# sergivalverde/sub-cortical_segmentation

Measured on NVIDIA B200. Metric: voxels_per_sec_full_volume_inference, higher is better.
Workload: dtype bf16

## Files before the change

sub-cortical_segmentation_b200/csrc/conv_sweep.cu:

```cuda
#include "tc_common.cuh"

namespace sc {

constexpr int SW_SLOT_HALF = 17408;
constexpr int SW_MAX_SLOTS = 14;
constexpr int SW_BAR_BYTES = 512;

struct SweepArgs {
  int Pw, R;
  int bn;
  int S;
  int nstrips, strip_w;
  int nseg, L;
  int n_items;
  int stages;
  int out_bufs;
  int npanels;
  int in_dx, in_dy;
  const float* scale; const float* shift; const float* alpha;
  unsigned long long* dbg;
  const uint8_t* item_on;
  double* stats;
  int st_H, st_pitch;
};

__device__ __forceinline__ void sweep_mma(uint32_t acc, uint32_t a_lo, uint32_t b_lo, uint32_t idesc, uint32_t accumulate, uint32_t elected) {
  asm volatile(
      "{\n\t"
      ".reg .pred p, q;\n\t"
      ".reg .b64 da, db;\n\t"
      "setp.ne.b32 p, %4, 0;\n\t"
      "setp.ne.b32 q, %5, 0;\n\t"
      "mov.b64 da, {%1, %6};\n\t"
      "mov.b64 db, {%2, %6};\n\t"
      "@q tcgen05.mma.cta_group::1.kind::f16 [%0], da, db, %3, p;\n\t"
      "}" ::"r"(acc), "r"(a_lo), "r"(b_lo), "r"(idesc), "r"(accumulate), "r"(elected), "r"(0x40004040u) : "memory");
}
__device__ __forceinline__ uint32_t desc_lo(uint32_t saddr) { return ((saddr & 0x3FFFFu) >> 4) | (1u << 16); }

__device__ __forceinline__ void tmem_ld16(uint32_t taddr, uint32_t (&r)[16]) {
  asm volatile(
      "tcgen05.ld.sync.aligned.32x32b.x16.b32 {%0, %1, %2, %3, %4, %5, %6, %7, %8, %9, %10, %11, %12, %13, %14, %15}, [%16];"
      : "=r"(r[0]), "=r"(r[1]), "=r"(r[2]), "=r"(r[3]), "=r"(r[4]), "=r"(r[5]), "=r"(r[6]), "=r"(r[7]), "=r"(r[8]),
        "=r"(r[9]), "=r"(r[10]), "=r"(r[11]), "=r"(r[12]), "=r"(r[13]), "=r"(r[14]), "=r"(r[15])
      : "r"(taddr));
}

__device__ __forceinline__ void tmem_ld8(uint32_t taddr, uint32_t (&r)[8]) {
  asm volatile("tcgen05.ld.sync.aligned.32x32b.x8.b32 {%0, %1, %2, %3, %4, %5, %6, %7}, [%8];"
               : "=r"(r[0]), "=r"(r[1]), "=r"(r[2]), "=r"(r[3]), "=r"(r[4]), "=r"(r[5]), "=r"(r[6]), "=r"(r[7])
               : "r"(taddr));
}
template <int CW>
__device__ __forceinline__ void sweep_stats_flush(float (&st_s)[CW], float (&st_q)[CW], float* s_red , int ew, int c0,
                                                  bool real, int lane, double* stats) {
#pragma unroll
  for (int k = 0; k < CW; ++k)
#pragma unroll
    for (int o = 16; o; o >>= 1) { st_s[k] += __shfl_xor_sync(0xffffffffu, st_s[k], o); st_q[k] += __shfl_xor_sync(0xffffffffu, st_q[k], o); }
  if (lane == 0) {
#pragma unroll
    for (int k = 0; k < CW; ++k) { s_red[ew * 2 * CW + k] = st_s[k]; s_red[ew * 2 * CW + CW + k] = st_q[k]; }
  }
  asm volatile("bar.sync 7, 512;" ::: "memory");
  if ((ew & 3) == 0 && real && lane < 2 * CW) {
    const int base = ew * 2 * CW + lane;
    const float tot = s_red[base] + s_red[base + 2 * CW] + s_red[base + 4 * CW] + s_red[base + 6 * CW];
    const int mom = lane / CW, ch = c0 + (lane - mom * CW);
    if (ch < 64) atomicAdd(&stats[ch * 2 + mom], (double)tot);
  }
}

template <int CW>
__device__ __forceinline__ void tmem_ld(uint32_t taddr, uint32_t (&r)[CW]) {
  if constexpr (CW == 16) tmem_ld16(taddr, r); else tmem_ld8(taddr, r);
}
template <int CW>
__device__ __forceinline__ void tmem_zero(uint32_t taddr) {
  if constexpr (CW == 16)
    asm volatile("tcgen05.st.sync.aligned.32x32b.x16.b32 [%0], {%1, %1, %1, %1, %1, %1, %1, %1, %1, %1, %1, %1, %1, %1, %1, %1};"
                 ::"r"(taddr), "r"(0u) : "memory");
  else
    asm volatile("tcgen05.st.sync.aligned.32x32b.x8.b32 [%0], {%1, %1, %1, %1, %1, %1, %1, %1};" ::"r"(taddr), "r"(0u) : "memory");
}
template <int CW>
__device__ __forceinline__ void sweep_acc_clear(uint32_t tcol, int S, int bn) {
  for (int j = 0; j < S + 2; ++j) tmem_zero<CW>(tcol + (uint32_t)(j * bn));
  asm volatile("tcgen05.wait::st.sync.aligned;" ::: "memory");
}
template <int CW, bool PAIR>
__device__ __forceinline__ void sweep_drain(uint64_t* afull, uint64_t* aempty, uint32_t& dj, uint32_t& dph, int S, int bn,
                                            uint32_t tcol, bool real, bool keep, int lane, float (&acc)[CW], bool timed,
                                            uint32_t& w_wait) {
  const long long c0 = timed ? clock64() : 0;
  mbar_wait(&afull[dj], (dph >> dj) & 1u);
  dph ^= 1u << dj;
  if (timed) w_wait += (uint32_t)(clock64() - c0);
  asm volatile("tcgen05.fence::after_thread_sync;" ::: "memory");
  if (real) {
    const uint32_t taddr = tcol + dj * (uint32_t)bn, tspill = taddr + (uint32_t)(S * bn);
    const bool split = dj < 2;
    if (keep) {
#pragma unroll
      for (int h = 0; h < CW; h += 8) {
        uint32_t r1[8], r2[8];
        tmem_ld8(taddr + h, r1);
        if (split) tmem_ld8(tspill + h, r2);
        asm volatile("tcgen05.wait::ld.sync.aligned;" ::: "memory");
#pragma unroll
        for (int k = 0; k < 8; ++k) acc[h + k] = split ? __uint_as_float(r1[k]) + __uint_as_float(r2[k]) : __uint_as_float(r1[k]);
      }
    }
    tmem_zero<CW>(taddr);
    if (split) tmem_zero<CW>(tspill);
    asm volatile("tcgen05.wait::st.sync.aligned;" ::: "memory");
  }
  asm volatile("tcgen05.fence::before_thread_sync;" ::: "memory");
  __syncwarp();
  if (lane == 0) {
    if (PAIR) mbar_arrive_cta(&aempty[dj], 0); else mbar_arrive(&aempty[dj]);
  }
  if (++dj == (uint32_t)S) dj = 0;
}
__device__ __forceinline__ void sweep_claim(uint64_t* aempty, uint32_t j, uint32_t& eph) {
  mbar_wait(&aempty[j], ((eph >> j) & 1u) ^ 1u);
  eph ^= 1u << j;
}
__device__ __forceinline__ uint32_t slot_back(uint32_t j, uint32_t k, int S) { return j >= k ? j - k : j + (uint32_t)S - k; }
__device__ __forceinline__ void tma_store_3d(const CUtensorMap* map, const void* src, int c0, int c1, int c2) {
  asm volatile("cp.async.bulk.tensor.3d.global.shared::cta.bulk_group [%0, {%2, %3, %4}], [%1];"
               ::"l"(reinterpret_cast<uint64_t>(map)), "r"(smem_u32(src)), "r"(c0), "r"(c1), "r"(c2) : "memory");
}
template <int KSTEPS, int DIL, int POOL, int CW, bool LO64, bool OUT32>
__global__ void __launch_bounds__(576, 1)
conv_sweep_kernel(const __grid_constant__ CUtensorMap mapA, const __grid_constant__ CUtensorMap mapW, const __grid_constant__ CUtensorMap mapO,
                  const SweepArgs a) {
  extern __shared__ uint8_t smem_raw[];
  uint8_t* smem = smem_raw + ((1024u - (smem_u32(smem_raw) & 1023u)) & 1023u);
  constexpr int BOXPX = 128 + 2 * DIL;
  constexpr int BOX_BYTES = BOXPX * 128;
  constexpr int NBOX = LO64 ? 1 : 2;
  constexpr int SLOT = NBOX * SW_SLOT_HALF;
  constexpr int LO_OFF = LO64 ? 64 : SW_SLOT_HALF;
  const int half_bytes = 3 * a.bn * 128;
  const int panel_bytes = 2 * half_bytes;
  const int w_bytes = a.npanels * panel_bytes;
  uint8_t* sW = smem;
  uint8_t* sRing = smem + w_bytes;
  constexpr int OB_BYTES = OUT32 ? 16384 : 32768;
  uint8_t* sOut = sRing + a.stages * SLOT;
  uint64_t* bars = reinterpret_cast<uint64_t*>(sOut + a.out_bufs * OB_BYTES);
  uint64_t* full = bars;
  uint64_t* empty = bars + a.stages;
  uint64_t* afull = bars + 2 * a.stages;
  uint64_t* aempty = afull + a.S;
  uint64_t* wfull = aempty + a.S;
  uint32_t* tmem_slot = reinterpret_cast<uint32_t*>(wfull + 1);
  float* s_const = reinterpret_cast<float*>(tmem_slot + 2);
  float* s_xch = s_const + 192;

  const int warp = threadIdx.x >> 5, lane = threadIdx.x & 31;

  if (threadIdx.x == 0) {
    for (int s = 0; s < a.stages; ++s) { mbar_init(&full[s], 1); mbar_init(&empty[s], 1); }
    for (int j = 0; j < a.S; ++j) { mbar_init(&afull[j], 1); mbar_init(&aempty[j], 16); }
    mbar_init(wfull, 1);
    asm volatile("fence.mbarrier_init.release.cluster;" ::: "memory");
  }
  if (warp == 1) {
    asm volatile("tcgen05.alloc.cta_group::1.sync.aligned.shared::cta.b32 [%0], %1;" ::"r"(smem_u32(tmem_slot)), "r"(512) : "memory");
    asm volatile("tcgen05.relinquish_alloc_permit.cta_group::1.sync.aligned;" ::: "memory");
  }
  for (int i = threadIdx.x; i < 64; i += blockDim.x) {
    const bool ok = i < a.bn;
    s_const[i] = ok ? __ldg(a.scale + i) : 0.f;
    s_const[64 + i] = ok ? __ldg(a.shift + i) : 0.f;
    s_const[128 + i] = ok ? __ldg(a.alpha + i) : 0.f;
  }
  for (int i = threadIdx.x; i < a.out_bufs * OB_BYTES / 16; i += blockDim.x)
    reinterpret_cast<uint4*>(sOut)[i] = make_uint4(0u, 0u, 0u, 0u);
  asm volatile("fence.proxy.async.shared::cta;" ::: "memory");
  asm volatile("tcgen05.fence::before_thread_sync;" ::: "memory");
  __syncthreads();
  asm volatile("tcgen05.fence::after_thread_sync;" ::: "memory");
  const uint32_t tmem_base = *tmem_slot;
  const int q4 = warp & 3, ew = warp - 2, grp = ew >> 2, c0 = grp * CW;
  const bool real = c0 < a.bn;
  const uint32_t tcol = tmem_base + ((uint32_t)(q4 * 32) << 16) + (uint32_t)c0;
  if (warp >= 2 && real) sweep_acc_clear<CW>(tcol, a.S, a.bn);
  asm volatile("tcgen05.fence::before_thread_sync;" ::: "memory");
  __syncthreads();
  asm volatile("tcgen05.fence::after_thread_sync;" ::: "memory");

  auto decode = [&](int item, int& w0, int& q, int& n0, int& Lc) {
    const int strip = item % a.nstrips;
    const int rest = item / a.nstrips;
    q = rest % DIL;
    const int seg = rest / DIL;
    w0 = strip * a.strip_w;
    const int Nq = (a.R - q + DIL - 1) / DIL;
    n0 = seg * a.L;
    Lc = Nq - n0 < a.L ? Nq - n0 : a.L;
  };

  if (warp == 0) {
    if (lane == 0) {
      asm volatile("prefetch.tensormap [%0];" ::"l"(reinterpret_cast<uint64_t>(&mapA)) : "memory");
      asm volatile("prefetch.tensormap [%0];" ::"l"(reinterpret_cast<uint64_t>(&mapW)) : "memory");
      asm volatile("prefetch.tensormap [%0];" ::"l"(reinterpret_cast<uint64_t>(&mapO)) : "memory");
      mbar_expect_tx(wfull, (uint32_t)w_bytes);
      for (int p = 0; p < 2 * a.npanels; ++p) tma_load_2d(&mapW, wfull, sW + p * half_bytes, 0, p * 3 * a.bn);
      uint32_t g = 0;
      long long w_empty = 0;
      const long long tstart = a.dbg ? clock64() : 0;
      for (int item = blockIdx.x; item < a.n_items; item += gridDim.x) {
        int w0, q, n0, Lc;
        decode(item, w0, q, n0, Lc);
        if (Lc <= 0 || (a.item_on && !a.item_on[item])) continue;
        const int nload = Lc + (POOL == 1 ? 1 : 0) + 2;
        for (int m = 0; m < nload; ++m, ++g) {
          const uint32_t s = g % a.stages, use = g / a.stages;
          if (use > 0) {
            const long long c0 = a.dbg ? clock64() : 0;
            mbar_wait(&empty[s], (use - 1) & 1);
            if (a.dbg) w_empty += clock64() - c0;
          }
          mbar_expect_tx(&full[s], (uint32_t)(NBOX * BOX_BYTES));
          uint8_t* sp = sRing + s * SLOT;
          const int r = q + DIL * (n0 + m);
          tma_load_3d(&mapA, &full[s], sp, 0, w0 + a.in_dx, r + a.in_dy);
          if (NBOX == 2) tma_load_3d(&mapA, &full[s], sp + SW_SLOT_HALF, 64, w0 + a.in_dx, r + a.in_dy);
        }
      }
      if (a.dbg) { a.dbg[blockIdx.x * 8 + 0] = (unsigned long long)w_empty; a.dbg[blockIdx.x * 8 + 1] = (unsigned long long)(clock64() - tstart); }
    }
    __syncwarp();
  } else if (warp == 1) {
    const uint32_t leader = elect_one();
    const uint32_t idesc = (1u << 4) | (1u << 7) | (1u << 10) | ((uint32_t)(3 * a.bn >> 3) << 17) | ((uint32_t)(128 >> 4) << 24);
    mbar_wait(wfull, 0);
    const uint32_t w_lo = desc_lo(smem_u32(sW));
    const uint32_t ring_lo = desc_lo(smem_u32(sRing));
    const uint32_t panel16 = (uint32_t)(panel_bytes >> 4), wl_off = (uint32_t)(half_bytes >> 4);
    uint32_t rs = 0, rph = 0;
    uint32_t j = 2, eph = 0;
    bool open = false;
    long long w_full = 0, w_tempty = 0;
    const long long tstart = a.dbg ? clock64() : 0;
    for (int item = blockIdx.x; item < a.n_items; item += gridDim.x) {
      int w0, q, n0, Lc;
      decode(item, w0, q, n0, Lc);
      if (Lc <= 0 || (a.item_on && !a.item_on[item])) continue;
      const int nin = Lc + (POOL == 1 ? 1 : 0) + 2;
      const uint32_t j0 = (uint32_t)(n0 + 2) % (uint32_t)a.S;
      const uint32_t d = open ? (j0 + (uint32_t)a.S - j) % (uint32_t)a.S : 2u;
      if (d) {
        if (open && leader) { umma_commit(&afull[slot_back(j, 2, a.S)]); if (d >= 2) umma_commit(&afull[slot_back(j, 1, a.S)]); }
        if (d >= 2) sweep_claim(aempty, slot_back(j0, 2, a.S), eph);
        sweep_claim(aempty, slot_back(j0, 1, a.S), eph);
      }
      j = j0; open = true;
      for (int m = 0; m < nin; ++m) {
        long long c0 = a.dbg ? clock64() : 0;
        sweep_claim(aempty, j, eph);
        if (a.dbg) { const long long c1 = clock64(); w_tempty += c1 - c0; c0 = c1; }
        mbar_wait(&full[rs], rph);
        if (a.dbg) w_full += clock64() - c0;
        asm volatile("tcgen05.fence::after_thread_sync;" ::: "memory");
        const uint32_t p = slot_back(j, 2, a.S);
        const uint32_t acc = tmem_base + p * (uint32_t)a.bn;
        const uint32_t sl = ring_lo + rs * (SLOT >> 4);
#pragma unroll
        for (int kx = 0; kx < 3; ++kx) {
#pragma unroll
          for (int ks = 0; ks < KSTEPS; ++ks) {
            const int gk = kx * KSTEPS + ks;
            const uint32_t a_hi = sl + (uint32_t)(kx * DIL * 8 + ks * 2);
            const uint32_t a_lo = a_hi + (uint32_t)(LO_OFF >> 4);
            const uint32_t wh = w_lo + (uint32_t)(gk >> 2) * panel16 + (uint32_t)((gk & 3) * 2);
            sweep_mma(acc, a_lo, wh, idesc, 1, leader);
            sweep_mma(acc, a_hi, wh + wl_off, idesc, 1, leader);
            sweep_mma(acc, a_hi, wh, idesc, 1, leader);
          }
        }
        if (leader) {
          umma_commit(&empty[rs]);
          umma_commit(&afull[p]);
        }
        __syncwarp();
        if (++rs == (uint32_t)a.stages) { rs = 0; rph ^= 1; }
        if (++j == (uint32_t)a.S) j = 0;
      }
    }
    if (open && leader) {
      umma_commit(&afull[slot_back(j, 2, a.S)]);
      umma_commit(&afull[slot_back(j, 1, a.S)]);
    }
    __syncwarp();
    if (a.dbg && leader) {
      a.dbg[blockIdx.x * 8 + 2] = (unsigned long long)w_full; a.dbg[blockIdx.x * 8 + 3] = (unsigned long long)w_tempty;
      a.dbg[blockIdx.x * 8 + 4] = (unsigned long long)(clock64() - tstart);
    }
  } else {
    const int px = q4 * 32 + lane;
    const bool issuer = threadIdx.x == 64;
    const int trow = POOL == 2 ? px >> 1 : px;
    const bool writer = POOL == 2 ? !(lane & 1) : true;
    const uint32_t row_off = (uint32_t)trow * 128u;
    const uint32_t sw = (uint32_t)(trow & 7);
    const uint32_t hi_chunk = (uint32_t)(c0 >> 3);
    const uint32_t lo_base = OUT32 ? 0u : 16384u, lo_chunk = OUT32 ? 4u + hi_chunk : hi_chunk;
    uint32_t t = 0, e = 0;
    uint32_t dj = 0, dph = 0;
    uint32_t w_tfull = 0;
    const bool timed = a.dbg != nullptr;
    const long long tstart = a.dbg ? clock64() : 0;
    constexpr bool STATS = POOL == 0 && DIL == 1;
    float st_s[STATS ? CW : 1], st_q[STATS ? CW : 1];
#pragma unroll
    for (int k = 0; k < (STATS ? CW : 1); ++k) st_s[k] = st_q[k] = 0.f;
    float v[CW];
    for (int item = blockIdx.x; item < a.n_items; item += gridDim.x) {
      int w0, q, n0, Lc;
      decode(item, w0, q, n0, Lc);
      if (Lc <= 0 || (a.item_on && !a.item_on[item])) continue;
      const int nrow = Lc + (POOL == 1 ? 1 : 0);
      const uint32_t j0 = (uint32_t)(n0 + 2) % (uint32_t)a.S;
      const uint32_t d = (j0 + 2u * (uint32_t)a.S - 2u - dj) % (uint32_t)a.S;
      if (t == 0 || d >= 3) {
        if (t > 0)
          for (int h = 0; h < 2; ++h) sweep_drain<CW, false>(afull, aempty, dj, dph, a.S, a.bn, tcol, real, false, lane, v, timed, w_tfull);
        dj = slot_back(j0, 2, a.S);
      } else {
        for (uint32_t h = 0; h < d; ++h) sweep_drain<CW, false>(afull, aempty, dj, dph, a.S, a.bn, tcol, real, false, lane, v, timed, w_tfull);
      }
      for (int h = 0; h < 2; ++h) sweep_drain<CW, false>(afull, aempty, dj, dph, a.S, a.bn, tcol, real, false, lane, v, timed, w_tfull);
      float hprev[CW];
#pragma unroll
      for (int k = 0; k < CW; ++k) hprev[k] = 0.f;
      for (int m = 0; m < nrow; ++m, ++t) {
        sweep_drain<CW, false>(afull, aempty, dj, dph, a.S, a.bn, tcol, real, true, lane, v, timed, w_tfull);
        if (real) {
#pragma unroll
          for (int k4 = 0; k4 < CW / 4; ++k4) {
            const float4 sc_ = *reinterpret_cast<const float4*>(s_const + c0 + 4 * k4);
            const float4 sh = *reinterpret_cast<const float4*>(s_const + 64 + c0 + 4 * k4);
            const float4 al = *reinterpret_cast<const float4*>(s_const + 128 + c0 + 4 * k4);
            v[4 * k4 + 0] = prelu(fmaf(v[4 * k4 + 0], sc_.x, sh.x), al.x);
            v[4 * k4 + 1] = prelu(fmaf(v[4 * k4 + 1], sc_.y, sh.y), al.y);
            v[4 * k4 + 2] = prelu(fmaf(v[4 * k4 + 2], sc_.z, sh.z), al.z);
            v[4 * k4 + 3] = prelu(fmaf(v[4 * k4 + 3], sc_.w, sh.w), al.w);
          }
        }

        int r_out = q + DIL * (n0 + m);
        if (POOL == 1) {
          if (real) {
            float* xw = s_xch + (((t & 1) * 4 + grp) * 4 + q4) * 32;
            if (lane < DIL) {
#pragma unroll
              for (int k4 = 0; k4 < CW / 4; ++k4)
                *reinterpret_cast<float4*>(xw + lane * 16 + 4 * k4) = make_float4(v[4 * k4], v[4 * k4 + 1], v[4 * k4 + 2], v[4 * k4 + 3]);
            }
            asm volatile("bar.sync %0, 128;" ::"r"(1 + grp) : "memory");
            const bool edge = lane >= 32 - DIL;
            const float* xr = s_xch + (((t & 1) * 4 + grp) * 4 + ((q4 + 1) & 3)) * 32 + (edge ? (lane - (32 - DIL)) * 16 : 0);
#pragma unroll
            for (int k4 = 0; k4 < CW / 4; ++k4) {
              const float4 x4 = *reinterpret_cast<const float4*>(xr + 4 * k4);
              const float xs[4] = {x4.x, x4.y, x4.z, x4.w};
#pragma unroll
              for (int k = 0; k < 4; ++k) {
                float nb = __shfl_down_sync(0xffffffffu, v[4 * k4 + k], DIL);
                if (edge) nb = xs[k];
                const float h = fmaxf(v[4 * k4 + k], nb);
                v[4 * k4 + k] = fmaxf(h, hprev[4 * k4 + k]);
                hprev[4 * k4 + k] = h;
              }
            }
          }
          if (m == 0) continue;
          r_out -= DIL;
        }
        if (POOL == 2) {
          if (real) {
#pragma unroll
            for (int k = 0; k < CW; ++k) {
              const float h = fmaxf(v[k], __shfl_down_sync(0xffffffffu, v[k], 1));
              v[k] = fmaxf(h, hprev[k]);
              hprev[k] = (m & 1) ? 0.f : h;
            }
          }
          if (!(m & 1)) continue;
          r_out >>= 1;
        }
        if constexpr (STATS) {
          if (a.stats && real) {
            const int wpx = w0 + px;
            if (wpx < a.Pw && (wpx & (a.st_pitch - 1)) < a.st_H && r_out < a.st_H) {
#pragma unroll
              for (int k = 0; k < CW; ++k) { st_s[k] += v[k]; st_q[k] = fmaf(v[k], v[k], st_q[k]); }
            }
          }
        }
        uint8_t* ob = sOut + (e % (uint32_t)a.out_bufs) * OB_BYTES;
        if (a.out_bufs == 1) {
          if (issuer) asm volatile("cp.async.bulk.wait_group.read 0;" ::: "memory");
          asm volatile("bar.sync 5, 512;" ::: "memory");
        }
        if (real) {
          uint32_t hi[CW / 2], lo[CW / 2];
#pragma unroll
          for (int k = 0; k < CW / 2; ++k) split2(v[2 * k], v[2 * k + 1], hi[k], lo[k]);
#pragma unroll
          for (int c = 0; c < CW / 8; ++c) {
            if (!writer) break;
            *reinterpret_cast<uint4*>(ob + row_off + (((hi_chunk + c) ^ sw) << 4)) = make_uint4(hi[4 * c], hi[4 * c + 1], hi[4 * c + 2], hi[4 * c + 3]);
            *reinterpret_cast<uint4*>(ob + lo_base + row_off + (((lo_chunk + c) ^ sw) << 4)) = make_uint4(lo[4 * c], lo[4 * c + 1], lo[4 * c + 2], lo[4 * c + 3]);
          }
          asm volatile("fence.proxy.async.shared::cta;" ::: "memory");
        }
        if (a.out_bufs == 2 && issuer) asm volatile("cp.async.bulk.wait_group.read 0;" ::: "memory");
        asm volatile("bar.sync 6, 512;" ::: "memory");
        if (issuer) {
          tma_store_3d(&mapO, ob, 0, POOL == 2 ? w0 >> 1 : w0, r_out);
          if (!OUT32) tma_store_3d(&mapO, ob + 16384, 64, POOL == 2 ? w0 >> 1 : w0, r_out);
          asm volatile("cp.async.bulk.commit_group;" ::: "memory");
        }
        ++e;
      }
    }
    if (t > 0)
      for (int h = 0; h < 2; ++h) sweep_drain<CW, false>(afull, aempty, dj, dph, a.S, a.bn, tcol, real, false, lane, v, timed, w_tfull);
    if (issuer) asm volatile("cp.async.bulk.wait_group 0;" ::: "memory");
    if constexpr (STATS) {
      if (a.stats) sweep_stats_flush<CW>(st_s, st_q, s_xch, ew, c0, real, lane, a.stats);
    }
    if (a.dbg && threadIdx.x == 64) {
      a.dbg[blockIdx.x * 8 + 5] = (unsigned long long)w_tfull; a.dbg[blockIdx.x * 8 + 6] = (unsigned long long)(clock64() - tstart);
      a.dbg[blockIdx.x * 8 + 7] = t;
    }
  }
  asm volatile("tcgen05.fence::before_thread_sync;" ::: "memory");
  __syncthreads();
  if (warp == 1) {
    asm volatile("tcgen05.fence::after_thread_sync;" ::: "memory");
    asm volatile("tcgen05.dealloc.cta_group::1.sync.aligned.b32 %0, %1;" ::"r"(tmem_base), "r"(512) : "memory");
  }
}

__device__ __forceinline__ void sweep_mma_2sm(uint32_t acc, uint32_t a_lo, uint32_t b_lo, uint32_t idesc, uint32_t accumulate, uint32_t elected) {
  asm volatile(
      "{\n\t"
      ".reg .pred p, q;\n\t"
      ".reg .b64 da, db;\n\t"
      "setp.ne.b32 p, %4, 0;\n\t"
      "setp.ne.b32 q, %5, 0;\n\t"
      "mov.b64 da, {%1, %6};\n\t"
      "mov.b64 db, {%2, %6};\n\t"
      "@q tcgen05.mma.cta_group::2.kind::f16 [%0], da, db, %3, p;\n\t"
      "}" ::"r"(acc), "r"(a_lo), "r"(b_lo), "r"(idesc), "r"(accumulate), "r"(elected), "r"(0x40004040u) : "memory");
}

template <int KSTEPS, int DIL, int POOL>
__global__ void __cluster_dims__(2, 1, 1) __launch_bounds__(576, 1)
conv_sweep_pair_kernel(const __grid_constant__ CUtensorMap mapA, const __grid_constant__ CUtensorMap mapW, const __grid_constant__ CUtensorMap mapO,
                       const SweepArgs a) {
  extern __shared__ uint8_t smem_raw[];
  uint8_t* smem = smem_raw + ((1024u - (smem_u32(smem_raw) & 1023u)) & 1023u);
  constexpr int BOXPX = 128 + 2 * DIL;
  constexpr int BOX_BYTES = BOXPX * 128;
  constexpr int SLOT = 2 * SW_SLOT_HALF;
  constexpr int CW = 16;
  const int panel_bytes = 3 * a.bn * 128;
  const int w_bytes = a.npanels * panel_bytes;
  uint8_t* sW = smem;
  uint8_t* sRing = smem + ((w_bytes + 1023) & ~1023);
  constexpr int OB_BYTES = 32768;
  uint8_t* sOut = sRing + a.stages * SLOT;
  uint64_t* bars = reinterpret_cast<uint64_t*>(sOut + a.out_bufs * OB_BYTES);
  uint64_t* full = bars;
  uint64_t* empty = bars + a.stages;
  uint64_t* afull = bars + 2 * a.stages;
  uint64_t* aempty = afull + a.S;
  uint64_t* wfull = aempty + a.S;
  uint32_t* tmem_slot = reinterpret_cast<uint32_t*>(wfull + 1);
  float* s_const = reinterpret_cast<float*>(tmem_slot + 2);
  float* s_xch = s_const + 192;

  const int warp = threadIdx.x >> 5, lane = threadIdx.x & 31;
  const uint32_t rank = cluster_ctarank();
  const int pair = blockIdx.x >> 1, npairs = gridDim.x >> 1;

  if (threadIdx.x == 0) {
    for (int s = 0; s < a.stages; ++s) { mbar_init(&full[s], 1); mbar_init(&empty[s], 1); }
    for (int j = 0; j < a.S; ++j) { mbar_init(&afull[j], 1); mbar_init(&aempty[j], 32); }
    mbar_init(wfull, 1);
    asm volatile("fence.mbarrier_init.release.cluster;" ::: "memory");
  }
  if (warp == 1) {
    asm volatile("tcgen05.alloc.cta_group::2.sync.aligned.shared::cta.b32 [%0], %1;" ::"r"(smem_u32(tmem_slot)), "r"(512) : "memory");
    asm volatile("tcgen05.relinquish_alloc_permit.cta_group::2.sync.aligned;" ::: "memory");
  }
  for (int i = threadIdx.x; i < 64; i += blockDim.x) {
    const bool ok = i < a.bn;
    s_const[i] = ok ? __ldg(a.scale + i) : 0.f;
    s_const[64 + i] = ok ? __ldg(a.shift + i) : 0.f;
    s_const[128 + i] = ok ? __ldg(a.alpha + i) : 0.f;
  }
  for (int i = threadIdx.x; i < a.out_bufs * OB_BYTES / 16; i += blockDim.x)
    reinterpret_cast<uint4*>(sOut)[i] = make_uint4(0u, 0u, 0u, 0u);
  asm volatile("fence.proxy.async.shared::cta;" ::: "memory");
  asm volatile("tcgen05.fence::before_thread_sync;" ::: "memory");
  __syncthreads();
  asm volatile("tcgen05.fence::after_thread_sync;" ::: "memory");
  const uint32_t tmem_base = *tmem_slot;
  const int q4 = warp & 3, ew = warp - 2, grp = ew >> 2, c0 = grp * CW;
  const bool real = c0 < a.bn;
  const uint32_t tcol = tmem_base + ((uint32_t)(q4 * 32) << 16) + (uint32_t)c0;
  if (warp >= 2 && real) sweep_acc_clear<CW>(tcol, a.S, a.bn);
  asm volatile("tcgen05.fence::before_thread_sync;" ::: "memory");
  __syncthreads();
  cluster_sync_all();
  asm volatile("tcgen05.fence::after_thread_sync;" ::: "memory");

  const int nsp = (a.nstrips + 1) >> 1;
  auto decode = [&](int item, int& w0, int& q, int& n0, int& Lc) {
    const int sp = item % nsp;
    const int rest = item / nsp;
    q = rest % DIL;
    const int seg = rest / DIL;
    w0 = (2 * sp + (int)rank) * a.strip_w;
    const int Nq = (a.R - q + DIL - 1) / DIL;
    n0 = seg * a.L;
    Lc = Nq - n0 < a.L ? Nq - n0 : a.L;
  };

  if (warp == 0) {
    if (lane == 0) {
      asm volatile("prefetch.tensormap [%0];" ::"l"(reinterpret_cast<uint64_t>(&mapA)) : "memory");
      asm volatile("prefetch.tensormap [%0];" ::"l"(reinterpret_cast<uint64_t>(&mapW)) : "memory");
      asm volatile("prefetch.tensormap [%0];" ::"l"(reinterpret_cast<uint64_t>(&mapO)) : "memory");
      {
        const uint32_t lbar = smem_u32(wfull) & 0xFEFFFFFFu;
        if (rank == 0) mbar_expect_tx(wfull, (uint32_t)(2 * w_bytes));
        for (int p = 0; p < a.npanels; ++p) tma_load_2d_2sm(&mapW, lbar, sW + p * panel_bytes, 0, (p * 2 + (int)rank) * 3 * a.bn);
      }
      uint32_t g = 0;
      long long w_empty = 0;
      const long long tstart = a.dbg ? clock64() : 0;
      for (int item = pair; item < a.n_items; item += npairs) {
        int w0, q, n0, Lc;
        decode(item, w0, q, n0, Lc);
        if (Lc <= 0 || (a.item_on && !a.item_on[item])) continue;
        const int nload = Lc + (POOL == 1 ? 1 : 0) + 2;
        for (int m = 0; m < nload; ++m, ++g) {
          const uint32_t s = g % a.stages, use = g / a.stages;
          if (use > 0) {
            const long long c0w = a.dbg ? clock64() : 0;
            mbar_wait(&empty[s], (use - 1) & 1);
            if (a.dbg) w_empty += clock64() - c0w;
          }
          const uint32_t lbar = smem_u32(&full[s]) & 0xFEFFFFFFu;
          if (rank == 0) mbar_expect_tx(&full[s], (uint32_t)(2 * 2 * BOX_BYTES));
          uint8_t* sp = sRing + s * SLOT;
          const int r = q + DIL * (n0 + m);
          tma_load_3d_2sm(&mapA, lbar, sp, 0, w0 + a.in_dx, r + a.in_dy);
          tma_load_3d_2sm(&mapA, lbar, sp + SW_SLOT_HALF, 64, w0 + a.in_dx, r + a.in_dy);
        }
      }
      if (a.dbg) { a.dbg[blockIdx.x * 8 + 0] = (unsigned long long)w_empty; a.dbg[blockIdx.x * 8 + 1] = (unsigned long long)(clock64() - tstart); }
    }
    __syncwarp();
  } else if (warp == 1) {
    if (rank == 0) {
      const uint32_t leader = elect_one();
      const uint32_t idesc = (1u << 4) | (1u << 7) | (1u << 10) | ((uint32_t)(3 * a.bn >> 3) << 17) | ((uint32_t)(256 >> 4) << 24);
      mbar_wait(wfull, 0);
      const uint32_t w_lo = desc_lo(smem_u32(sW));
      const uint32_t ring_lo = desc_lo(smem_u32(sRing));
      const uint32_t panel16 = (uint32_t)(panel_bytes >> 4);
      const uint32_t wl_off = (uint32_t)(3 * a.bn / 2 * 128) >> 4;
      uint32_t rs = 0, rph = 0, j = 2, eph = 0;
      bool open = false;
      long long w_full = 0, w_tempty = 0;
      const long long tstart = a.dbg ? clock64() : 0;
      for (int item = pair; item < a.n_items; item += npairs) {
        int w0, q, n0, Lc;
        decode(item, w0, q, n0, Lc);
        if (Lc <= 0 || (a.item_on && !a.item_on[item])) continue;
        const int nin = Lc + (POOL == 1 ? 1 : 0) + 2;
        const uint32_t j0 = (uint32_t)(n0 + 2) % (uint32_t)a.S;
        const uint32_t d = open ? (j0 + (uint32_t)a.S - j) % (uint32_t)a.S : 2u;
        if (d) {
          if (open && leader) { umma_commit_2sm(&afull[slot_back(j, 2, a.S)]); if (d >= 2) umma_commit_2sm(&afull[slot_back(j, 1, a.S)]); }
          if (d >= 2) sweep_claim(aempty, slot_back(j0, 2, a.S), eph);
          sweep_claim(aempty, slot_back(j0, 1, a.S), eph);
        }
        j = j0; open = true;
        for (int m = 0; m < nin; ++m) {
          long long c0w = a.dbg ? clock64() : 0;
          sweep_claim(aempty, j, eph);
          if (a.dbg) { const long long c1 = clock64(); w_tempty += c1 - c0w; c0w = c1; }
          mbar_wait(&full[rs], rph);
          if (a.dbg) w_full += clock64() - c0w;
          asm volatile("tcgen05.fence::after_thread_sync;" ::: "memory");
          const uint32_t p = slot_back(j, 2, a.S);
          const uint32_t acc = tmem_base + p * (uint32_t)a.bn;
          const uint32_t sl = ring_lo + rs * (SLOT >> 4);
#pragma unroll
          for (int kx = 0; kx < 3; ++kx) {
#pragma unroll
            for (int ks = 0; ks < KSTEPS; ++ks) {
              const int gk = kx * KSTEPS + ks;
              const uint32_t a_hi = sl + (uint32_t)(kx * DIL * 8 + ks * 2);
              const uint32_t a_lo = a_hi + (uint32_t)(SW_SLOT_HALF >> 4);
              const uint32_t wh = w_lo + (uint32_t)(gk >> 2) * panel16 + (uint32_t)((gk & 3) * 2);
              sweep_mma_2sm(acc, a_lo, wh, idesc, 1, leader);
              sweep_mma_2sm(acc, a_hi, wh + wl_off, idesc, 1, leader);
              sweep_mma_2sm(acc, a_hi, wh, idesc, 1, leader);
            }
          }
          if (leader) {
            umma_commit_2sm(&empty[rs]);
            umma_commit_2sm(&afull[p]);
          }
          __syncwarp();
          if (++rs == (uint32_t)a.stages) { rs = 0; rph ^= 1; }
          if (++j == (uint32_t)a.S) j = 0;
        }
      }
      if (open && leader) {
        umma_commit_2sm(&afull[slot_back(j, 2, a.S)]);
        umma_commit_2sm(&afull[slot_back(j, 1, a.S)]);
      }
      __syncwarp();
      if (a.dbg && leader) {
        a.dbg[blockIdx.x * 8 + 2] = (unsigned long long)w_full; a.dbg[blockIdx.x * 8 + 3] = (unsigned long long)w_tempty;
        a.dbg[blockIdx.x * 8 + 4] = (unsigned long long)(clock64() - tstart);
      }
    }
  } else {
    const int px = q4 * 32 + lane;
    const bool issuer = threadIdx.x == 64;
    const int trow = POOL == 2 ? px >> 1 : px;
    const bool writer = POOL == 2 ? !(lane & 1) : true;
    const uint32_t row_off = (uint32_t)trow * 128u;
    const uint32_t sw = (uint32_t)(trow & 7);
    const uint32_t hi_chunk = (uint32_t)(c0 >> 3);
    uint32_t t = 0, e = 0, dj = 0, dph = 0;
    uint32_t w_tfull = 0;
    const bool timed = a.dbg != nullptr;
    const long long tstart = a.dbg ? clock64() : 0;
    constexpr bool STATS = POOL == 0 && DIL == 1;
    float st_s[STATS ? CW : 1], st_q[STATS ? CW : 1];
#pragma unroll
    for (int k = 0; k < (STATS ? CW : 1); ++k) st_s[k] = st_q[k] = 0.f;
    float v[CW];
    for (int item = pair; item < a.n_items; item += npairs) {
      int w0, q, n0, Lc;
      decode(item, w0, q, n0, Lc);
      if (Lc <= 0 || (a.item_on && !a.item_on[item])) continue;
      const int nrow = Lc + (POOL == 1 ? 1 : 0);
      const uint32_t j0 = (uint32_t)(n0 + 2) % (uint32_t)a.S;
      const uint32_t d = (j0 + 2u * (uint32_t)a.S - 2u - dj) % (uint32_t)a.S;
      if (t == 0 || d >= 3) {
        if (t > 0)
          for (int h = 0; h < 2; ++h) sweep_drain<CW, true>(afull, aempty, dj, dph, a.S, a.bn, tcol, real, false, lane, v, timed, w_tfull);
        dj = slot_back(j0, 2, a.S);
      } else {
        for (uint32_t h = 0; h < d; ++h) sweep_drain<CW, true>(afull, aempty, dj, dph, a.S, a.bn, tcol, real, false, lane, v, timed, w_tfull);
      }
      for (int h = 0; h < 2; ++h) sweep_drain<CW, true>(afull, aempty, dj, dph, a.S, a.bn, tcol, real, false, lane, v, timed, w_tfull);
      float hprev[CW];
#pragma unroll
      for (int k = 0; k < CW; ++k) hprev[k] = 0.f;
      for (int m = 0; m < nrow; ++m, ++t) {
        sweep_drain<CW, true>(afull, aempty, dj, dph, a.S, a.bn, tcol, real, true, lane, v, timed, w_tfull);
        if (real) {
#pragma unroll
          for (int k4 = 0; k4 < CW / 4; ++k4) {
            const float4 sc_ = *reinterpret_cast<const float4*>(s_const + c0 + 4 * k4);
            const float4 sh = *reinterpret_cast<const float4*>(s_const + 64 + c0 + 4 * k4);
            const float4 al = *reinterpret_cast<const float4*>(s_const + 128 + c0 + 4 * k4);
            v[4 * k4 + 0] = prelu(fmaf(v[4 * k4 + 0], sc_.x, sh.x), al.x);
            v[4 * k4 + 1] = prelu(fmaf(v[4 * k4 + 1], sc_.y, sh.y), al.y);
            v[4 * k4 + 2] = prelu(fmaf(v[4 * k4 + 2], sc_.z, sh.z), al.z);
            v[4 * k4 + 3] = prelu(fmaf(v[4 * k4 + 3], sc_.w, sh.w), al.w);
          }
        }

        int r_out = q + DIL * (n0 + m);
        if (POOL == 1) {
          if (real) {
            float* xw = s_xch + (((t & 1) * 4 + grp) * 4 + q4) * 32;
            if (lane < DIL) {
#pragma unroll
              for (int k4 = 0; k4 < CW / 4; ++k4)
                *reinterpret_cast<float4*>(xw + lane * 16 + 4 * k4) = make_float4(v[4 * k4], v[4 * k4 + 1], v[4 * k4 + 2], v[4 * k4 + 3]);
            }
            asm volatile("bar.sync %0, 128;" ::"r"(1 + grp) : "memory");
            const bool edge = lane >= 32 - DIL;
            const float* xr = s_xch + (((t & 1) * 4 + grp) * 4 + ((q4 + 1) & 3)) * 32 + (edge ? (lane - (32 - DIL)) * 16 : 0);
#pragma unroll
            for (int k4 = 0; k4 < CW / 4; ++k4) {
              const float4 x4 = *reinterpret_cast<const float4*>(xr + 4 * k4);
              const float xs[4] = {x4.x, x4.y, x4.z, x4.w};
#pragma unroll
              for (int k = 0; k < 4; ++k) {
                float nb = __shfl_down_sync(0xffffffffu, v[4 * k4 + k], DIL);
                if (edge) nb = xs[k];
                const float h = fmaxf(v[4 * k4 + k], nb);
                v[4 * k4 + k] = fmaxf(h, hprev[4 * k4 + k]);
                hprev[4 * k4 + k] = h;
              }
            }
          }
          if (m == 0) continue;
          r_out -= DIL;
        }
        if (POOL == 2) {
          if (real) {
#pragma unroll
            for (int k = 0; k < CW; ++k) {
              const float h = fmaxf(v[k], __shfl_down_sync(0xffffffffu, v[k], 1));
              v[k] = fmaxf(h, hprev[k]);
              hprev[k] = (m & 1) ? 0.f : h;
            }
          }
          if (!(m & 1)) continue;
          r_out >>= 1;
        }
        if constexpr (STATS) {
          if (a.stats && real) {
            const int wpx = w0 + px;
            if (wpx < a.Pw && (wpx & (a.st_pitch - 1)) < a.st_H && r_out < a.st_H) {
#pragma unroll
              for (int k = 0; k < CW; ++k) { st_s[k] += v[k]; st_q[k] = fmaf(v[k], v[k], st_q[k]); }
            }
          }
        }
        uint8_t* ob = sOut + (e % (uint32_t)a.out_bufs) * OB_BYTES;
        if (a.out_bufs == 1) {
          if (issuer) asm volatile("cp.async.bulk.wait_group.read 0;" ::: "memory");
          asm volatile("bar.sync 5, 512;" ::: "memory");
        }
        if (real) {
          uint32_t hi[CW / 2], lo[CW / 2];
#pragma unroll
          for (int k = 0; k < CW / 2; ++k) split2(v[2 * k], v[2 * k + 1], hi[k], lo[k]);
#pragma unroll
          for (int c = 0; c < CW / 8; ++c) {
            if (!writer) break;
            *reinterpret_cast<uint4*>(ob + row_off + (((hi_chunk + c) ^ sw) << 4)) = make_uint4(hi[4 * c], hi[4 * c + 1], hi[4 * c + 2], hi[4 * c + 3]);
            *reinterpret_cast<uint4*>(ob + 16384 + row_off + (((hi_chunk + c) ^ sw) << 4)) = make_uint4(lo[4 * c], lo[4 * c + 1], lo[4 * c + 2], lo[4 * c + 3]);
          }
          asm volatile("fence.proxy.async.shared::cta;" ::: "memory");
        }
        if (a.out_bufs == 2 && issuer) asm volatile("cp.async.bulk.wait_group.read 0;" ::: "memory");
        asm volatile("bar.sync 6, 512;" ::: "memory");
        if (issuer) {
          tma_store_3d(&mapO, ob, 0, POOL == 2 ? w0 >> 1 : w0, r_out);
          tma_store_3d(&mapO, ob + 16384, 64, POOL == 2 ? w0 >> 1 : w0, r_out);
          asm volatile("cp.async.bulk.commit_group;" ::: "memory");
        }
        ++e;
      }
    }
    if (t > 0)
      for (int h = 0; h < 2; ++h) sweep_drain<CW, true>(afull, aempty, dj, dph, a.S, a.bn, tcol, real, false, lane, v, timed, w_tfull);
    if (issuer) asm volatile("cp.async.bulk.wait_group 0;" ::: "memory");
    if constexpr (STATS) {
      if (a.stats) sweep_stats_flush<CW>(st_s, st_q, s_xch, ew, c0, real, lane, a.stats);
    }
    if (a.dbg && threadIdx.x == 64) {
      a.dbg[blockIdx.x * 8 + 5] = (unsigned long long)w_tfull; a.dbg[blockIdx.x * 8 + 6] = (unsigned long long)(clock64() - tstart);
      a.dbg[blockIdx.x * 8 + 7] = t;
    }
  }
  asm volatile("tcgen05.fence::before_thread_sync;" ::: "memory");
  __syncthreads();
  cluster_sync_all();
  if (warp == 1) {
    asm volatile("tcgen05.fence::after_thread_sync;" ::: "memory");
    asm volatile("tcgen05.dealloc.cta_group::2.sync.aligned.b32 %0, %1;" ::"r"(tmem_base), "r"(512) : "memory");
  }
}

__device__ __forceinline__ void tma_store_4d(const CUtensorMap* map, const void* src, int c0, int c1, int c2, int c3) {
  asm volatile("cp.async.bulk.tensor.4d.global.shared::cta.bulk_group [%0, {%2, %3, %4, %5}], [%1];"
               ::"l"(reinterpret_cast<uint64_t>(map)), "r"(smem_u32(src)), "r"(c0), "r"(c1), "r"(c2), "r"(c3) : "memory");
}

__global__ void __launch_bounds__(256) conv1_wide_kernel(const __grid_constant__ CUtensorMap mapO, const __grid_constant__ Conv1Consts cw,
                                                         const float* __restrict__ vol, ViewGeo g, int ns, int outR, int outC, int slice_fast) {
  extern __shared__ uint8_t smem_raw[];
  uint8_t* tiles = smem_raw + ((1024u - (smem_u32(smem_raw) & 1023u)) & 1023u);
  const int bc = slice_fast ? 8 : 32, bs = slice_fast ? 32 : 8;
  const int nct = (outC + bc - 1) / bc, nst = (ns + bs - 1) / bs;
  const long long n_tiles = (long long)outR * nst * nct;
  const int f = threadIdx.x & 31, sl = threadIdx.x >> 5;
  const int cl = slice_fast ? sl : f, sloc = slice_fast ? f : sl;
  const int trow = sloc * bc + cl;
  const uint32_t row_off = (uint32_t)trow * 128u, swz = (uint32_t)(trow & 7);
  uint32_t it = 0;
  for (long long t = blockIdx.x; t < n_tiles; t += gridDim.x, ++it) {
    const int ct = (int)(t % nct);
    const int stl = (int)((t / nct) % nst);
    const int i = (int)(t / ((long long)nct * nst));
    const int j = ct * bc + cl, s = stl * bs + sloc;
    uint8_t* ob = tiles + (it & 1) * 32768;
    if (it >= 2) {
      if (threadIdx.x == 0) asm volatile("cp.async.bulk.wait_group.read 1;" ::: "memory");
      __syncthreads();
    }
    float v[20];
    if (j < outC && s < ns) {
      const float* vb = vol + (int64_t)(g.s0 + s) * g.ss;
      float x[9];
#pragma unroll
      for (int ky = 0; ky < 3; ++ky) {
        const int rr = g.r0 + i + ky - 16;
#pragma unroll
        for (int kx = 0; kx < 3; ++kx) {
          const int cc = g.c0 + j + kx - 16;
          x[ky * 3 + kx] = (rr >= 0 && rr < g.R && cc >= 0 && cc < g.C) ? __ldg(vb + (int64_t)rr * g.rs + (int64_t)cc * g.cs) : 0.f;
        }
      }
#pragma unroll
      for (int co = 0; co < 20; ++co) {
        float acc = 0.f;
#pragma unroll
        for (int tp = 0; tp < 9; ++tp) acc = fmaf(x[tp], cw.w[tp * 20 + co], acc);
        v[co] = prelu(fmaf(acc, cw.scale[co], cw.shift[co]), cw.alpha[co]);
      }
    } else {
#pragma unroll
      for (int co = 0; co < 20; ++co) v[co] = 0.f;
    }
    uint32_t hi[12], lo[12];
#pragma unroll
    for (int k = 0; k < 10; ++k) split2(v[2 * k], v[2 * k + 1], hi[k], lo[k]);
    hi[10] = hi[11] = lo[10] = lo[11] = 0u;
#pragma unroll
    for (int c = 0; c < 3; ++c) {
      *reinterpret_cast<uint4*>(ob + row_off + (((uint32_t)c ^ swz) << 4)) = make_uint4(hi[4 * c], hi[4 * c + 1], hi[4 * c + 2], hi[4 * c + 3]);
      *reinterpret_cast<uint4*>(ob + row_off + (((uint32_t)(4 + c) ^ swz) << 4)) = make_uint4(lo[4 * c], lo[4 * c + 1], lo[4 * c + 2], lo[4 * c + 3]);
    }
    *reinterpret_cast<uint4*>(ob + row_off + ((3u ^ swz) << 4)) = make_uint4(0u, 0u, 0u, 0u);
    *reinterpret_cast<uint4*>(ob + row_off + ((7u ^ swz) << 4)) = make_uint4(0u, 0u, 0u, 0u);
    asm volatile("fence.proxy.async.shared::cta;" ::: "memory");
    __syncthreads();
    if (threadIdx.x == 0) {
      tma_store_4d(&mapO, ob, 0, ct * bc, stl * bs, i);
      asm volatile("cp.async.bulk.commit_group;" ::: "memory");
    }
  }
  if (threadIdx.x == 0) asm volatile("cp.async.bulk.wait_group 0;" ::: "memory");
}

int launch_conv1_wide(sc_ctx* ctx, const float* vol, const ViewGeo& g, int ns, const Conv1Consts& cw, float* out, int outR, int outC,
                      cudaStream_t st) {
  TcState* s = reinterpret_cast<TcState*>(ctx->tc_state);
  SC_CHECK(s != nullptr, SC_ERR_UNSUPPORTED, "tcgen05 back-end not initialised");
  if (ns <= 0 || outR <= 0 || outC <= 0) return SC_OK;
  const int slice_fast = (g.ss == 1 && g.cs != 1) ? 1 : 0;
  const int bc = slice_fast ? 8 : 32, bs = slice_fast ? 32 : 8;
  CUtensorMap mapO;
  cuuint64_t dims[4] = {64, (cuuint64_t)outC, (cuuint64_t)ns, (cuuint64_t)outR};
  cuuint64_t strides[3] = {128, (cuuint64_t)outC * 128, (cuuint64_t)ns * outC * 128};
  cuuint32_t box[4] = {64, (cuuint32_t)bc, (cuuint32_t)bs, 1};
  cuuint32_t es[4] = {1, 1, 1, 1};
  CUresult r = s->encode(&mapO, CU_TENSOR_MAP_DATA_TYPE_BFLOAT16, 4, out, dims, strides, box, es, CU_TENSOR_MAP_INTERLEAVE_NONE,
                         CU_TENSOR_MAP_SWIZZLE_128B, CU_TENSOR_MAP_L2_PROMOTION_NONE, CU_TENSOR_MAP_FLOAT_OOB_FILL_NONE);
  SC_CHECK(r == CUDA_SUCCESS, SC_ERR_CUDA, "conv1_wide: cuTensorMapEncodeTiled failed with %d", (int)r);
  SC_TRY(ensure_smem_attr(ctx, reinterpret_cast<const void*>(conv1_wide_kernel), 2 * 32768 + 1024));
  const long long n_tiles = (long long)outR * ((ns + bs - 1) / bs) * ((outC + bc - 1) / bc);
  const long long cap = (long long)ctx->sm_count * 3;
  const unsigned grid = (unsigned)(n_tiles < cap ? n_tiles : cap);
  ProfScope prof(ctx, PC_CONV1, st);
  conv1_wide_kernel<<<grid, 256, 2 * 32768 + 1024, st>>>(mapO, cw, vol, g, ns, outR, outC, slice_fast);
  ctx->launches++;
  SC_CUDA(cudaGetLastError());
  return SC_OK;
}

template <int KSTEPS, int DIL, int POOL, int CW, bool LO64, bool OUT32>
static int launch_sweep_t(sc_ctx* ctx, const CUtensorMap& mapA, const CUtensorMap& mapW, const CUtensorMap& mapO, const SweepArgs& a,
                          size_t smem, cudaStream_t st) {
  auto kern = conv_sweep_kernel<KSTEPS, DIL, POOL, CW, LO64, OUT32>;
  SC_TRY(ensure_smem_attr(ctx, reinterpret_cast<const void*>(kern), 227 * 1024));
  const int grid = a.n_items < ctx->sm_count ? a.n_items : ctx->sm_count;
  kern<<<grid, 576, smem, st>>>(mapA, mapW, mapO, a);
  ctx->launches++;
  SC_CUDA(cudaGetLastError());
  return SC_OK;
}

__global__ void __launch_bounds__(256) view_occupancy_kernel(const uint8_t* __restrict__ cand, ViewGeo g, uint32_t* __restrict__ occ) {
  const int64_t w = (int64_t)blockIdx.x * 8 + (threadIdx.x >> 5);
  if (w >= (int64_t)g.br * g.ns) return;
  const int lane = threadIdx.x & 31;
  const int i = (int)(w / g.ns), sl = (int)(w - (int64_t)i * g.ns);
  const uint8_t* base = cand + (int64_t)(g.s0 + sl) * g.ss + (int64_t)(g.r0 + i) * g.rs + (int64_t)g.c0 * g.cs;
  uint32_t bits = 0;
  for (int jb = 0; jb * 32 < g.bc; ++jb) {
    const int j = jb * 32 + lane;
    const bool on = j < g.bc && base[(int64_t)j * g.cs] != 0;
    if (__any_sync(0xffffffffu, on)) bits |= 1u << jb;
  }
  if (lane == 0) occ[w] = bits;
}

int launch_view_occupancy(sc_ctx* ctx, const uint8_t* cand, const ViewGeo& g, uint32_t* occ, cudaStream_t st) {
  SC_CHECK(g.bc <= 1024, SC_ERR_ARG, "sweep skip: more than 1024 columns per slice");
  const int64_t warps = (int64_t)g.br * g.ns;
  view_occupancy_kernel<<<(unsigned)((warps + 7) / 8), 256, 0, st>>>(cand, g, occ);
  ctx->launches++;
  SC_CUDA(cudaGetLastError());
  return SC_OK;
}

__global__ void __launch_bounds__(256) sweep_item_flags_kernel(const uint32_t* __restrict__ occ, int br, int bc, int ns, int C1, int reach, int n_items,
                                                               int nstr, int dil, int L, int R, int item_w, int Pw, uint8_t* __restrict__ flags) {
  const int item = blockIdx.x * 8 + (threadIdx.x >> 5);
  if (item >= n_items) return;
  const int lane = threadIdx.x & 31;
  const int strip = item % nstr, rest = item / nstr;
  const int q = rest % dil, seg = rest / dil;
  const int Nq = (R - q + dil - 1) / dil;
  const int n0 = seg * L;
  const int Lc = Nq - n0 < L ? Nq - n0 : L;
  bool any = false;
  if (Lc > 0) {
    const int rlo = q + dil * n0, rhi = q + dil * (n0 + Lc - 1);
    const int ilo = rlo - reach > 0 ? rlo - reach : 0, ihi = rhi < br - 1 ? rhi : br - 1;
    const int w0 = strip * item_w;
    int w1 = w0 + item_w - 1;
    if (w1 > Pw - 1) w1 = Pw - 1;
    if (w0 <= w1 && ilo <= ihi) {
      const int sa = w0 / C1, sb = w1 / C1;
      const int nrow = ihi - ilo + 1;
      for (int e = lane; e < nrow * (sb - sa + 1); e += 32) {
        const int sl = sa + e / nrow, i = ilo + e % nrow;
        if (sl >= ns) continue;
        const int clo = w0 - sl * C1 > 0 ? w0 - sl * C1 : 0;
        const int chi = w1 - sl * C1 < C1 - 1 ? w1 - sl * C1 : C1 - 1;
        const int jlo = clo - reach > 0 ? clo - reach : 0, jhi = chi < bc - 1 ? chi : bc - 1;
        if (jlo > jhi) continue;
        const int b0 = jlo >> 5, b1 = jhi >> 5;
        const uint32_t colmask = (b1 - b0 == 31 ? 0xffffffffu : ((1u << (b1 - b0 + 1)) - 1u)) << b0;
        if (occ[(int64_t)i * ns + sl] & colmask) any = true;
      }
    }
  }
  any = __any_sync(0xffffffffu, any);
  if (lane == 0) flags[item] = any ? 1 : 0;
}

static int launch_item_flags(sc_ctx* ctx, const SweepSkip* skip, SweepArgs& a, int nstr, int item_w, int dil, int rows_out, cudaStream_t st) {
  if (!skip) return SC_OK;
  sweep_item_flags_kernel<<<(unsigned)((a.n_items + 7) / 8), 256, 0, st>>>(skip->occ, skip->br, skip->bc, skip->ns, skip->C1, rows_out - skip->br,
                                                                         a.n_items, nstr, dil, a.L, a.R, item_w, a.Pw, skip->flags);
  ctx->launches++;
  SC_CUDA(cudaGetLastError());
  a.item_on = skip->flags;
  return SC_OK;
}

int launch_conv_sweep(sc_ctx* ctx, const SweepW& w, int layer, const float* in, int in_fmt, float* out, int out_fmt,
                      int Pw, int R, int rows_out, int dil, int pool, int prof_cls, cudaStream_t st, int in_dx, int in_dy, const SweepSkip* skip,
                      const SweepStats* stats) {
  TcState* s = reinterpret_cast<TcState*>(ctx->tc_state);
  SC_CHECK(s != nullptr, SC_ERR_UNSUPPORTED, "tcgen05 back-end not initialised");
  if (Pw <= 0 || R <= 0) return SC_OK;
  SweepArgs a;
  if (rows_out <= 0 || rows_out > R) rows_out = R;
  a.Pw = Pw; a.R = rows_out; a.bn = w.bn;
  a.strip_w = 128 - (pool == 1 ? dil : 0);
  a.nstrips = (Pw + a.strip_w - 1) / a.strip_w;
  const int nq = (rows_out + dil - 1) / dil;
  int nseg = (4 * ctx->sm_count + a.nstrips * dil - 1) / (a.nstrips * dil);
  int L = (nq + nseg - 1) / nseg;
  if (L < 12) L = 12;
  if (a.nstrips * dil * ((nq + 11) / 12) < ctx->sm_count) {
    nseg = (ctx->sm_count + a.nstrips * dil - 1) / (a.nstrips * dil);
    L = (nq + nseg - 1) / nseg;
    if (L < 2) L = 2;
  }
  if (L > 96) L = 96;
  if (skip && L > 32) L = 32;
  if (pool == 2) L = (L + 1) & ~1;
  nseg = (nq + L - 1) / L;
  a.L = L; a.nseg = nseg;
  a.n_items = a.nstrips * dil * nseg;
  a.item_on = nullptr;
  a.stats = nullptr; a.st_H = 0; a.st_pitch = 1;
  if (stats) {
    SC_CHECK(dil == 1 && !pool && (stats->pitch & (stats->pitch - 1)) == 0, SC_ERR_ARG, "conv_sweep: fused statistics need dil 1, no pool, a power-of-two pitch");
    a.stats = stats->sums; a.st_H = stats->H; a.st_pitch = stats->pitch;
  }
  SC_CHECK(pool != 2 || dil == 1, SC_ERR_ARG, "conv_sweep: the stride-2 pool needs dilation 1");
  a.npanels = w.npanels;
  a.in_dx = in_dx; a.in_dy = in_dy;
  a.scale = w.scale; a.shift = w.shift; a.alpha = w.alpha;
  a.dbg = (ctx->tc_timing_cls == prof_cls) ? ctx->tc_timing_buf : nullptr;
  SC_CHECK(w.bn <= (out_fmt ? 32 : 64) && w.bn % 16 == 0, SC_ERR_ARG, "conv_sweep: bad channel geometry");
  a.S = 512 / w.bn - 2;
  if (a.S > SW_MAX_SLOTS) a.S = SW_MAX_SLOTS;
  const int slot = (in_fmt ? 1 : 2) * SW_SLOT_HALF;
  const int w_bytes = w.npanels * 6 * w.bn * 128;
  const int ob_bytes = out_fmt ? 16384 : 32768;
  const int fixed = 1024 + w_bytes + SW_BAR_BYTES + 192 * 4 + 2 * 4 * 4 * 2 * 16 * 4;
  a.out_bufs = 2;
  a.stages = (227 * 1024 - fixed - 2 * ob_bytes) / slot;
  if (a.stages < 3) {
    a.out_bufs = 1;
    a.stages = (227 * 1024 - fixed - ob_bytes) / slot;
  }
  if (a.stages > 8) a.stages = 8;
  const bool use_pair = w.ksteps >= 3 && !in_fmt && !out_fmt;
  SC_CHECK(use_pair || a.stages >= 2, SC_ERR_ARG, "conv_sweep: ring does not fit (layer %d)", layer);
  const size_t smem = (size_t)fixed + (size_t)a.stages * slot + (size_t)a.out_bufs * ob_bytes;

  CUtensorMap mapA, mapW, mapO;
  {
    const int pxe = in_fmt ? 64 : 128;
    cuuint64_t dims[3] = {(cuuint64_t)pxe, (cuuint64_t)Pw, (cuuint64_t)R};
    cuuint64_t strides[2] = {(cuuint64_t)pxe * 2, (cuuint64_t)Pw * pxe * 2};
    cuuint32_t box[3] = {64, (cuuint32_t)(128 + 2 * dil), 1};
    cuuint32_t es[3] = {1, 1, 1};
    CUresult r = s->encode(&mapA, CU_TENSOR_MAP_DATA_TYPE_BFLOAT16, 3, const_cast<float*>(in), dims, strides, box, es,
                           CU_TENSOR_MAP_INTERLEAVE_NONE, CU_TENSOR_MAP_SWIZZLE_128B, CU_TENSOR_MAP_L2_PROMOTION_L2_256B,
                           CU_TENSOR_MAP_FLOAT_OOB_FILL_NONE);
    SC_CHECK(r == CUDA_SUCCESS, SC_ERR_CUDA, "conv_sweep: cuTensorMapEncodeTiled(A) failed with %d (Pw %d R %d)", (int)r, Pw, R);
  }
  {
    cuuint64_t dims[2] = {64, (cuuint64_t)w.npanels * 6 * w.bn};
    cuuint64_t strides[1] = {128};
    cuuint32_t box[2] = {64, (cuuint32_t)(3 * w.bn)};
    cuuint32_t es[2] = {1, 1};
    CUresult r = s->encode(&mapW, CU_TENSOR_MAP_DATA_TYPE_BFLOAT16, 2, w.panels, dims, strides, box, es,
                           CU_TENSOR_MAP_INTERLEAVE_NONE, CU_TENSOR_MAP_SWIZZLE_128B, CU_TENSOR_MAP_L2_PROMOTION_L2_256B,
                           CU_TENSOR_MAP_FLOAT_OOB_FILL_NONE);
    SC_CHECK(r == CUDA_SUCCESS, SC_ERR_CUDA, "conv_sweep: cuTensorMapEncodeTiled(W) failed with %d", (int)r);
  }
  {
    const int pxe = out_fmt ? 64 : 128;
    const int oPw = pool == 2 ? Pw / 2 : Pw, oR = pool == 2 ? R / 2 : R;
    cuuint64_t dims[3] = {(cuuint64_t)pxe, (cuuint64_t)oPw, (cuuint64_t)oR};
    cuuint64_t strides[2] = {(cuuint64_t)pxe * 2, (cuuint64_t)oPw * pxe * 2};
    cuuint32_t box[3] = {64, (cuuint32_t)(pool == 2 ? 64 : a.strip_w), 1};
    cuuint32_t es[3] = {1, 1, 1};
    CUresult r = s->encode(&mapO, CU_TENSOR_MAP_DATA_TYPE_BFLOAT16, 3, out, dims, strides, box, es,
                           CU_TENSOR_MAP_INTERLEAVE_NONE, CU_TENSOR_MAP_SWIZZLE_128B, CU_TENSOR_MAP_L2_PROMOTION_NONE,
                           CU_TENSOR_MAP_FLOAT_OOB_FILL_NONE);
    SC_CHECK(r == CUDA_SUCCESS, SC_ERR_CUDA, "conv_sweep: cuTensorMapEncodeTiled(O) failed with %d", (int)r);
  }
  const bool i32 = in_fmt != 0, o32 = out_fmt != 0;
  if (use_pair) {
    const int nsp = (a.nstrips + 1) / 2;
    const int pairs_max = ctx->sm_count / 2;
    nseg = (4 * pairs_max + nsp * dil - 1) / (nsp * dil);
    L = (nq + nseg - 1) / nseg;
    if (L < 12) L = 12;
    if (nsp * dil * ((nq + 11) / 12) < pairs_max) {
      nseg = (pairs_max + nsp * dil - 1) / (nsp * dil);
      L = (nq + nseg - 1) / nseg;
      if (L < 2) L = 2;
    }
    if (L > 96) L = 96;
    if (skip && L > 32) L = 32;
    if (pool == 2) L = (L + 1) & ~1;
    nseg = (nq + L - 1) / L;
    a.L = L; a.nseg = nseg;
    a.n_items = nsp * dil * nseg;
    const int wp_bytes = w.npanels * 3 * w.bn * 128;
    const int fixed_p = 1024 + ((wp_bytes + 1023) & ~1023) + SW_BAR_BYTES + 192 * 4 + ((pool || stats) ? 2 * 4 * 4 * 2 * 16 * 4 : 0);
    a.out_bufs = 2;
    a.stages = (227 * 1024 - fixed_p - 2 * ob_bytes) / slot;
    if (a.stages < 3) { a.out_bufs = 1; a.stages = (227 * 1024 - fixed_p - ob_bytes) / slot; }
    if (a.stages > 8) a.stages = 8;
    SC_CHECK(a.stages >= 2, SC_ERR_ARG, "conv_sweep: pair ring does not fit (layer %d)", layer);
    SC_CHECK(pool != 2 || (Pw % 2 == 0), SC_ERR_ARG, "conv_sweep: odd pitch with the stride-2 pool");
    const size_t smem_p = (size_t)fixed_p + (size_t)a.stages * slot + (size_t)a.out_bufs * ob_bytes;
    CUtensorMap mapWp;
    cuuint64_t dims[2] = {64, (cuuint64_t)w.npanels * 6 * w.bn};
    cuuint64_t strides[1] = {128};
    cuuint32_t box[2] = {64, (cuuint32_t)(3 * w.bn)};
    cuuint32_t es[2] = {1, 1};
    CUresult r = s->encode(&mapWp, CU_TENSOR_MAP_DATA_TYPE_BFLOAT16, 2, w.panels_pair, dims, strides, box, es,
                           CU_TENSOR_MAP_INTERLEAVE_NONE, CU_TENSOR_MAP_SWIZZLE_128B, CU_TENSOR_MAP_L2_PROMOTION_L2_256B,
                           CU_TENSOR_MAP_FLOAT_OOB_FILL_NONE);
    SC_CHECK(r == CUDA_SUCCESS, SC_ERR_CUDA, "conv_sweep: cuTensorMapEncodeTiled(W pair) failed with %d", (int)r);
    const int npairs = a.n_items < pairs_max ? a.n_items : pairs_max;
    SC_TRY(launch_item_flags(ctx, skip, a, nsp, 2 * a.strip_w, dil, rows_out, st));
    ProfScope prof(ctx, prof_cls, st);
    if (dil == 1 && pool == 2) {
      auto kern = conv_sweep_pair_kernel<3, 1, 2>;
      SC_TRY(ensure_smem_attr(ctx, reinterpret_cast<const void*>(kern), 227 * 1024));
      kern<<<2 * npairs, 576, smem_p, st>>>(mapA, mapWp, mapO, a);
    } else if (dil == 1 && !pool && w.ksteps == 4) {
      auto kern = conv_sweep_pair_kernel<4, 1, 0>;
      SC_TRY(ensure_smem_attr(ctx, reinterpret_cast<const void*>(kern), 227 * 1024));
      kern<<<2 * npairs, 576, smem_p, st>>>(mapA, mapWp, mapO, a);
    } else if (dil == 1 && !pool) {
      auto kern = conv_sweep_pair_kernel<3, 1, 0>;
      SC_TRY(ensure_smem_attr(ctx, reinterpret_cast<const void*>(kern), 227 * 1024));
      kern<<<2 * npairs, 576, smem_p, st>>>(mapA, mapWp, mapO, a);
    } else if (dil == 2 && pool == 1) {
      auto kern = conv_sweep_pair_kernel<3, 2, 1>;
      SC_TRY(ensure_smem_attr(ctx, reinterpret_cast<const void*>(kern), 227 * 1024));
      kern<<<2 * npairs, 576, smem_p, st>>>(mapA, mapWp, mapO, a);
    } else if (dil == 4 && !pool) {
      auto kern = conv_sweep_pair_kernel<3, 4, 0>;
      SC_TRY(ensure_smem_attr(ctx, reinterpret_cast<const void*>(kern), 227 * 1024));
      kern<<<2 * npairs, 576, smem_p, st>>>(mapA, mapWp, mapO, a);
    } else {
      set_error("conv_sweep: no pair kernel instance for dil=%d pool=%d", dil, pool);
      return SC_ERR_ARG;
    }
    ctx->launches++;
    SC_CUDA(cudaGetLastError());
    return SC_OK;
  }
  SC_TRY(launch_item_flags(ctx, skip, a, a.nstrips, a.strip_w, dil, rows_out, st));
  ProfScope prof(ctx, prof_cls, st);
  if (w.ksteps == 2 && dil == 1 && pool == 2 && i32 && o32 && w.bn == 32) return launch_sweep_t<2, 1, 2, 8, true, true>(ctx, mapA, mapW, mapO, a, smem, st);
  if (w.ksteps == 2 && dil == 1 && pool == 1 && i32 && o32 && w.bn == 32) return launch_sweep_t<2, 1, 1, 8, true, true>(ctx, mapA, mapW, mapO, a, smem, st);
  if (w.ksteps == 2 && dil == 2 && !pool && i32 && !o32) return launch_sweep_t<2, 2, 0, 16, true, false>(ctx, mapA, mapW, mapO, a, smem, st);
  if (w.ksteps == 2 && dil == 1 && !pool && i32 && !o32) return launch_sweep_t<2, 1, 0, 16, true, false>(ctx, mapA, mapW, mapO, a, smem, st);
  if (w.ksteps == 2 && dil == 1 && !pool && i32 && o32 && w.bn == 32) return launch_sweep_t<2, 1, 0, 8, true, true>(ctx, mapA, mapW, mapO, a, smem, st);
  set_error("conv_sweep: no kernel instance for ksteps=%d dil=%d pool=%d in_fmt=%d out_fmt=%d", w.ksteps, dil, pool, in_fmt, out_fmt);
  return SC_ERR_ARG;
}

}
```

Baseline: 164.6 million.

## Replace CTA-wide epilogue barriers with per-quarter stores and deferred TMEM slot release

The epilogue no longer synchronises all 512 consumer threads before each output TMA store. Each 128-thread quarter now uses its own named barrier and issues its own narrower TMA store, with a separate tensor map for the last quarter when pooling shrinks it. The pool-1 neighbour exchange swaps the group bar.sync for per-box mbarriers, and the TMEM slot release is deferred to the next drain so its store-wait overlaps other work. In exchange there are four times as many small TMA stores, extra mbarrier bookkeeping, and more complex ordering that could introduce hazards.

Result: no change. 164.1 million, median of 6 (-0.3%).

```diff
diff --git a/sub-cortical_segmentation_b200/csrc/conv_sweep.cu b/sub-cortical_segmentation_b200/csrc/conv_sweep.cu
--- a/sub-cortical_segmentation_b200/csrc/conv_sweep.cu
+++ b/sub-cortical_segmentation_b200/csrc/conv_sweep.cu
@@ -88,53 +88,133 @@
   for (int j = 0; j < S + 2; ++j) tmem_zero<CW>(tcol + (uint32_t)(j * bn));
   asm volatile("tcgen05.wait::st.sync.aligned;" ::: "memory");
 }
+__device__ __forceinline__ void tma_store_3d(const CUtensorMap* map, const void* src, int c0, int c1, int c2) {
+  asm volatile("cp.async.bulk.tensor.3d.global.shared::cta.bulk_group [%0, {%2, %3, %4}], [%1];"
+               ::"l"(reinterpret_cast<uint64_t>(map)), "r"(smem_u32(src)), "r"(c0), "r"(c1), "r"(c2) : "memory");
+}
+__device__ __forceinline__ uint32_t slot_back(uint32_t j, uint32_t k, int S) { return j >= k ? j - k : j + (uint32_t)S - k; }
+template <bool PAIR>
+__device__ __forceinline__ void sweep_release(uint64_t* aempty, uint32_t dj, bool& pend, int S, int lane) {
+  if (!pend) return;
+  asm volatile("tcgen05.wait::st.sync.aligned;" ::: "memory");
+  asm volatile("tcgen05.fence::before_thread_sync;" ::: "memory");
+  __syncwarp();
+  if (lane == 0) {
+    const uint32_t j = slot_back(dj, 1, S);
+    if (PAIR) mbar_arrive_cta(&aempty[j], 0); else mbar_arrive(&aempty[j]);
+  }
+  pend = false;
+}
 template <int CW, bool PAIR>
-__device__ __forceinline__ void sweep_drain(uint64_t* afull, uint64_t* aempty, uint32_t& dj, uint32_t& dph, int S, int bn,
+__device__ __forceinline__ void sweep_drain(uint64_t* afull, uint64_t* aempty, uint32_t& dj, uint32_t& dph, bool& pend, int S, int bn,
                                             uint32_t tcol, bool real, bool keep, int lane, float (&acc)[CW], bool timed,
-                                            uint32_t& w_wait) {
+                                            uint32_t* w_wait) {
+  sweep_release<PAIR>(aempty, dj, pend, S, lane);
   const long long c0 = timed ? clock64() : 0;
   mbar_wait(&afull[dj], (dph >> dj) & 1u);
   dph ^= 1u << dj;
-  if (timed) w_wait += (uint32_t)(clock64() - c0);
+  if (timed) *w_wait += (uint32_t)(clock64() - c0);
   asm volatile("tcgen05.fence::after_thread_sync;" ::: "memory");
   if (real) {
     const uint32_t taddr = tcol + dj * (uint32_t)bn, tspill = taddr + (uint32_t)(S * bn);
     const bool split = dj < 2;
-    if (keep) {
+    if (keep && !split) {
+      uint32_t r[CW];
+      tmem_ld<CW>(taddr, r);
+      asm volatile("tcgen05.wait::ld.sync.aligned;" ::: "memory");
+#pragma unroll
+      for (int k = 0; k < CW; ++k) acc[k] = __uint_as_float(r[k]);
+    } else if (keep) {
 #pragma unroll
       for (int h = 0; h < CW; h += 8) {
         uint32_t r1[8], r2[8];
         tmem_ld8(taddr + h, r1);
-        if (split) tmem_ld8(tspill + h, r2);
+        tmem_ld8(tspill + h, r2);
         asm volatile("tcgen05.wait::ld.sync.aligned;" ::: "memory");
 #pragma unroll
-        for (int k = 0; k < 8; ++k) acc[h + k] = split ? __uint_as_float(r1[k]) + __uint_as_float(r2[k]) : __uint_as_float(r1[k]);
+        for (int k = 0; k < 8; ++k) acc[h + k] = __uint_as_float(r1[k]) + __uint_as_float(r2[k]);
       }
     }
     tmem_zero<CW>(taddr);
     if (split) tmem_zero<CW>(tspill);
-    asm volatile("tcgen05.wait::st.sync.aligned;" ::: "memory");
-  }
-  asm volatile("tcgen05.fence::before_thread_sync;" ::: "memory");
-  __syncwarp();
-  if (lane == 0) {
-    if (PAIR) mbar_arrive_cta(&aempty[dj], 0); else mbar_arrive(&aempty[dj]);
-  }
+  }
+  pend = true;
   if (++dj == (uint32_t)S) dj = 0;
+}
+template <int CW, int DIL>
+__device__ __forceinline__ void sweep_pool1(float (&v)[CW], float (&hprev)[CW], float* s_xch, uint64_t* xbar, uint32_t t, int grp, int q4,
+                                            int lane) {
+  const int box = (int)((t & 1u) * 4u + (uint32_t)grp) * 4;
+  const uint32_t use = t >> 1;
+  if (q4 > 0) {
+    if (use > 0) mbar_wait(&xbar[32 + box + q4], (use - 1u) & 1u);
+    if (lane < DIL) {
+      float* xw = s_xch + (box + q4) * 32 + lane * 16;
+#pragma unroll
+      for (int k4 = 0; k4 < CW / 4; ++k4)
+        *reinterpret_cast<float4*>(xw + 4 * k4) = make_float4(v[4 * k4], v[4 * k4 + 1], v[4 * k4 + 2], v[4 * k4 + 3]);
+      mbar_arrive(&xbar[box + q4]);
+    }
+  }
+  const bool edge = q4 < 3 && lane >= 32 - DIL;
+  if (q4 < 3) mbar_wait(&xbar[box + q4 + 1], use & 1u);
+  const float* xr = s_xch + (box + q4 + 1) * 32 + (lane - (32 - DIL)) * 16;
+#pragma unroll
+  for (int k4 = 0; k4 < CW / 4; ++k4) {
+    const float4 x4 = edge ? *reinterpret_cast<const float4*>(xr + 4 * k4) : make_float4(0.f, 0.f, 0.f, 0.f);
+    const float xs[4] = {x4.x, x4.y, x4.z, x4.w};
+#pragma unroll
+    for (int k = 0; k < 4; ++k) {
+      float nb = __shfl_down_sync(0xffffffffu, v[4 * k4 + k], DIL);
+      if (edge) nb = xs[k];
+      const float h = fmaxf(v[4 * k4 + k], nb);
+      v[4 * k4 + k] = fmaxf(h, hprev[4 * k4 + k]);
+      hprev[4 * k4 + k] = h;
+    }
+  }
+  if (edge) mbar_arrive(&xbar[32 + box + q4 + 1]);
+}
+template <int CW, int DIL, int POOL, bool OUT32>
+__device__ __forceinline__ void sweep_emit(const float (&v)[CW], uint8_t* ob, int out_bufs, bool real, bool writer, uint32_t row_off,
+                                           uint32_t sw, uint32_t hi_chunk, int q4, bool qissuer, const CUtensorMap* mapO,
+                                           const CUtensorMap* mapO3, int wq, int r_out) {
+  constexpr uint32_t LO_BASE = OUT32 ? 0u : 16384u, LO_CHUNK = OUT32 ? 4u : 0u;
+  constexpr int QPX = POOL == 2 ? 16 : 32;
+  const int bar = 1 + q4;
+  if (out_bufs == 1) {
+    if (qissuer) asm volatile("cp.async.bulk.wait_group.read 0;" ::: "memory");
+    asm volatile("bar.sync %0, 128;" ::"r"(bar) : "memory");
+  }
+  if (real) {
+    uint32_t hi[CW / 2], lo[CW / 2];
+#pragma unroll
+    for (int k = 0; k < CW / 2; ++k) split2(v[2 * k], v[2 * k + 1], hi[k], lo[k]);
+#pragma unroll
+    for (int c = 0; c < CW / 8; ++c) {
+      if (!writer) break;
+      *reinterpret_cast<uint4*>(ob + row_off + (((hi_chunk + c) ^ sw) << 4)) = make_uint4(hi[4 * c], hi[4 * c + 1], hi[4 * c + 2], hi[4 * c + 3]);
+      *reinterpret_cast<uint4*>(ob + LO_BASE + row_off + (((LO_CHUNK + hi_chunk + c) ^ sw) << 4)) = make_uint4(lo[4 * c], lo[4 * c + 1], lo[4 * c + 2], lo[4 * c + 3]);
+    }
+    asm volatile("fence.proxy.async.shared::cta;" ::: "memory");
+  }
+  if (out_bufs == 2 && qissuer) asm volatile("cp.async.bulk.wait_group.read 0;" ::: "memory");
+  asm volatile("bar.sync %0, 128;" ::"r"(bar) : "memory");
+  if (qissuer) {
+    const CUtensorMap* m = (POOL == 1 && q4 == 3) ? mapO3 : mapO;
+    const uint8_t* src = ob + q4 * QPX * 128;
+    tma_store_3d(m, src, 0, wq, r_out);
+    if (!OUT32) tma_store_3d(m, src + 16384, 64, wq, r_out);
+    asm volatile("cp.async.bulk.commit_group;" ::: "memory");
+  }
 }
 __device__ __forceinline__ void sweep_claim(uint64_t* aempty, uint32_t j, uint32_t& eph) {
   mbar_wait(&aempty[j], ((eph >> j) & 1u) ^ 1u);
   eph ^= 1u << j;
 }
-__device__ __forceinline__ uint32_t slot_back(uint32_t j, uint32_t k, int S) { return j >= k ? j - k : j + (uint32_t)S - k; }
-__device__ __forceinline__ void tma_store_3d(const CUtensorMap* map, const void* src, int c0, int c1, int c2) {
-  asm volatile("cp.async.bulk.tensor.3d.global.shared::cta.bulk_group [%0, {%2, %3, %4}], [%1];"
-               ::"l"(reinterpret_cast<uint64_t>(map)), "r"(smem_u32(src)), "r"(c0), "r"(c1), "r"(c2) : "memory");
-}
 template <int KSTEPS, int DIL, int POOL, int CW, bool LO64, bool OUT32>
 __global__ void __launch_bounds__(576, 1)
 conv_sweep_kernel(const __grid_constant__ CUtensorMap mapA, const __grid_constant__ CUtensorMap mapW, const __grid_constant__ CUtensorMap mapO,
-                  const SweepArgs a) {
+                  const __grid_constant__ CUtensorMap mapO3, const SweepArgs a) {
   extern __shared__ uint8_t smem_raw[];
   uint8_t* smem = smem_raw + ((1024u - (smem_u32(smem_raw) & 1023u)) & 1023u);
   constexpr int BOXPX = 128 + 2 * DIL;
@@ -158,12 +238,15 @@
   uint32_t* tmem_slot = reinterpret_cast<uint32_t*>(wfull + 1);
   float* s_const = reinterpret_cast<float*>(tmem_slot + 2);
   float* s_xch = s_const + 192;
+  uint64_t* xbar = reinterpret_cast<uint64_t*>(s_xch + 1024);
 
   const int warp = threadIdx.x >> 5, lane = threadIdx.x & 31;
 
   if (threadIdx.x == 0) {
     for (int s = 0; s < a.stages; ++s) { mbar_init(&full[s], 1); mbar_init(&empty[s], 1); }
     for (int j = 0; j < a.S; ++j) { mbar_init(&afull[j], 1); mbar_init(&aempty[j], 16); }
+    if (POOL == 1)
+      for (int i = 0; i < 64; ++i) mbar_init(&xbar[i], DIL);
     mbar_init(wfull, 1);
     asm volatile("fence.mbarrier_init.release.cluster;" ::: "memory");
   }
@@ -208,6 +291,7 @@
       asm volatile("prefetch.tensormap [%0];" ::"l"(reinterpret_cast<uint64_t>(&mapA)) : "memory");
       asm volatile("prefetch.tensormap [%0];" ::"l"(reinterpret_cast<uint64_t>(&mapW)) : "memory");
       asm volatile("prefetch.tensormap [%0];" ::"l"(reinterpret_cast<uint64_t>(&mapO)) : "memory");
+      if (POOL == 1) asm volatile("prefetch.tensormap [%0];" ::"l"(reinterpret_cast<uint64_t>(&mapO3)) : "memory");
       mbar_expect_tx(wfull, (uint32_t)w_bytes);
       for (int p = 0; p < 2 * a.npanels; ++p) tma_load_2d(&mapW, wfull, sW + p * half_bytes, 0, p * 3 * a.bn);
       uint32_t g = 0;
@@ -303,18 +387,19 @@
     }
   } else {
     const int px = q4 * 32 + lane;
-    const bool issuer = threadIdx.x == 64;
+    const bool qissuer = grp == 0 && lane == 0;
     const int trow = POOL == 2 ? px >> 1 : px;
     const bool writer = POOL == 2 ? !(lane & 1) : true;
     const uint32_t row_off = (uint32_t)trow * 128u;
     const uint32_t sw = (uint32_t)(trow & 7);
     const uint32_t hi_chunk = (uint32_t)(c0 >> 3);
-    const uint32_t lo_base = OUT32 ? 0u : 16384u, lo_chunk = OUT32 ? 4u + hi_chunk : hi_chunk;
     uint32_t t = 0, e = 0;
     uint32_t dj = 0, dph = 0;
-    uint32_t w_tfull = 0;
-    const bool timed = a.dbg != nullptr;
-    const long long tstart = a.dbg ? clock64() : 0;
+    bool pend = false;
+    uint32_t* w_tfull = tmem_slot + 1;
+    const bool timed = a.dbg != nullptr && threadIdx.x == 64;
+    if (timed) *w_tfull = 0u;
+    if (a.dbg && threadIdx.x == 64) a.dbg[blockIdx.x * 8 + 6] = (unsigned long long)clock64();
     constexpr bool STATS = POOL == 0 && DIL == 1;
     float st_s[STATS ? CW : 1], st_q[STATS ? CW : 1];
 #pragma unroll
@@ -329,17 +414,18 @@
       const uint32_t d = (j0 + 2u * (uint32_t)a.S - 2u - dj) % (uint32_t)a.S;
       if (t == 0 || d >= 3) {
         if (t > 0)
-          for (int h = 0; h < 2; ++h) sweep_drain<CW, false>(afull, aempty, dj, dph, a.S, a.bn, tcol, real, false, lane, v, timed, w_tfull);
+          for (int h = 0; h < 2; ++h) sweep_drain<CW, false>(afull, aempty, dj, dph, pend, a.S, a.bn, tcol, real, false, lane, v, timed, w_tfull);
+        sweep_release<false>(aempty, dj, pend, a.S, lane);
         dj = slot_back(j0, 2, a.S);
       } else {
-        for (uint32_t h = 0; h < d; ++h) sweep_drain<CW, false>(afull, aempty, dj, dph, a.S, a.bn, tcol, real, false, lane, v, timed, w_tfull);
-      }
-      for (int h = 0; h < 2; ++h) sweep_drain<CW, false>(afull, aempty, dj, dph, a.S, a.bn, tcol, real, false, lane, v, timed, w_tfull);
+        for (uint32_t h = 0; h < d; ++h) sweep_drain<CW, false>(afull, aempty, dj, dph, pend, a.S, a.bn, tcol, real, false, lane, v, timed, w_tfull);
+      }
+      for (int h = 0; h < 2; ++h) sweep_drain<CW, false>(afull, aempty, dj, dph, pend, a.S, a.bn, tcol, real, false, lane, v, timed, w_tfull);
       float hprev[CW];
 #pragma unroll
       for (int k = 0; k < CW; ++k) hprev[k] = 0.f;
       for (int m = 0; m < nrow; ++m, ++t) {
-        sweep_drain<CW, false>(afull, aempty, dj, dph, a.S, a.bn, tcol, real, true, lane, v, timed, w_tfull);
+        sweep_drain<CW, false>(afull, aempty, dj, dph, pend, a.S, a.bn, tcol, real, true, lane, v, timed, w_tfull);
         if (real) {
 #pragma unroll
           for (int k4 = 0; k4 < CW / 4; ++k4) {
@@ -355,30 +441,7 @@
 
         int r_out = q + DIL * (n0 + m);
         if (POOL == 1) {
-          if (real) {
-            float* xw = s_xch + (((t & 1) * 4 + grp) * 4 + q4) * 32;
-            if (lane < DIL) {
-#pragma unroll
-              for (int k4 = 0; k4 < CW / 4; ++k4)
-                *reinterpret_cast<float4*>(xw + lane * 16 + 4 * k4) = make_float4(v[4 * k4], v[4 * k4 + 1], v[4 * k4 + 2], v[4 * k4 + 3]);
-            }
-            asm volatile("bar.sync %0, 128;" ::"r"(1 + grp) : "memory");
-            const bool edge = lane >= 32 - DIL;
-            const float* xr = s_xch + (((t & 1) * 4 + grp) * 4 + ((q4 + 1) & 3)) * 32 + (edge ? (lane - (32 - DIL)) * 16 : 0);
-#pragma unroll
-            for (int k4 = 0; k4 < CW / 4; ++k4) {
-              const float4 x4 = *reinterpret_cast<const float4*>(xr + 4 * k4);
-              const float xs[4] = {x4.x, x4.y, x4.z, x4.w};
-#pragma unroll
-              for (int k = 0; k < 4; ++k) {
-                float nb = __shfl_down_sync(0xffffffffu, v[4 * k4 + k], DIL);
-                if (edge) nb = xs[k];
-                const float h = fmaxf(v[4 * k4 + k], nb);
-                v[4 * k4 + k] = fmaxf(h, hprev[4 * k4 + k]);
-                hprev[4 * k4 + k] = h;
-              }
-            }
-          }
+          if (real) sweep_pool1<CW, DIL>(v, hprev, s_xch, xbar, t, grp, q4, lane);
           if (m == 0) continue;
           r_out -= DIL;
         }
@@ -403,41 +466,20 @@
             }
           }
         }
-        uint8_t* ob = sOut + (e % (uint32_t)a.out_bufs) * OB_BYTES;
-        if (a.out_bufs == 1) {
-          if (issuer) asm volatile("cp.async.bulk.wait_group.read 0;" ::: "memory");
-          asm volatile("bar.sync 5, 512;" ::: "memory");
-        }
-        if (real) {
-          uint32_t hi[CW / 2], lo[CW / 2];
-#pragma unroll
-          for (int k = 0; k < CW / 2; ++k) split2(v[2 * k], v[2 * k + 1], hi[k], lo[k]);
-#pragma unroll
-          for (int c = 0; c < CW / 8; ++c) {
-            if (!writer) break;
-            *reinterpret_cast<uint4*>(ob + row_off + (((hi_chunk + c) ^ sw) << 4)) = make_uint4(hi[4 * c], hi[4 * c + 1], hi[4 * c + 2], hi[4 * c + 3]);
-            *reinterpret_cast<uint4*>(ob + lo_base + row_off + (((lo_chunk + c) ^ sw) << 4)) = make_uint4(lo[4 * c], lo[4 * c + 1], lo[4 * c + 2], lo[4 * c + 3]);
-          }
-          asm volatile("fence.proxy.async.shared::cta;" ::: "memory");
-        }
-        if (a.out_bufs == 2 && issuer) asm volatile("cp.async.bulk.wait_group.read 0;" ::: "memory");
-        asm volatile("bar.sync 6, 512;" ::: "memory");
-        if (issuer) {
-          tma_store_3d(&mapO, ob, 0, POOL == 2 ? w0 >> 1 : w0, r_out);
-          if (!OUT32) tma_store_3d(&mapO, ob + 16384, 64, POOL == 2 ? w0 >> 1 : w0, r_out);
-          asm volatile("cp.async.bulk.commit_group;" ::: "memory");
-        }
+        sweep_emit<CW, DIL, POOL, OUT32>(v, sOut + (e % (uint32_t)a.out_bufs) * OB_BYTES, a.out_bufs, real, writer, row_off, sw, hi_chunk,
+                                         q4, qissuer, &mapO, &mapO3, (POOL == 2 ? w0 >> 1 : w0) + q4 * (POOL == 2 ? 16 : 32), r_out);
         ++e;
       }
     }
     if (t > 0)
-      for (int h = 0; h < 2; ++h) sweep_drain<CW, false>(afull, aempty, dj, dph, a.S, a.bn, tcol, real, false, lane, v, timed, w_tfull);
-    if (issuer) asm volatile("cp.async.bulk.wait_group 0;" ::: "memory");
+      for (int h = 0; h < 2; ++h) sweep_drain<CW, false>(afull, aempty, dj, dph, pend, a.S, a.bn, tcol, real, false, lane, v, timed, w_tfull);
+    sweep_release<false>(aempty, dj, pend, a.S, lane);
+    if (qissuer) asm volatile("cp.async.bulk.wait_group 0;" ::: "memory");
     if constexpr (STATS) {
       if (a.stats) sweep_stats_flush<CW>(st_s, st_q, s_xch, ew, c0, real, lane, a.stats);
     }
     if (a.dbg && threadIdx.x == 64) {
-      a.dbg[blockIdx.x * 8 + 5] = (unsigned long long)w_tfull; a.dbg[blockIdx.x * 8 + 6] = (unsigned long long)(clock64() - tstart);
+      a.dbg[blockIdx.x * 8 + 5] = (unsigned long long)*w_tfull; a.dbg[blockIdx.x * 8 + 6] = (unsigned long long)clock64() - a.dbg[blockIdx.x * 8 + 6];
       a.dbg[blockIdx.x * 8 + 7] = t;
     }
   }
@@ -465,7 +507,7 @@
 template <int KSTEPS, int DIL, int POOL>
 __global__ void __cluster_dims__(2, 1, 1) __launch_bounds__(576, 1)
 conv_sweep_pair_kernel(const __grid_constant__ CUtensorMap mapA, const __grid_constant__ CUtensorMap mapW, const __grid_constant__ CUtensorMap mapO,
-                       const SweepArgs a) {
+                       const __grid_constant__ CUtensorMap mapO3, const SweepArgs a) {
   extern __shared__ uint8_t smem_raw[];
   uint8_t* smem = smem_raw + ((1024u - (smem_u32(smem_raw) & 1023u)) & 1023u);
   constexpr int BOXPX = 128 + 2 * DIL;
@@ -487,6 +529,7 @@
   uint32_t* tmem_slot = reinterpret_cast<uint32_t*>(wfull + 1);
   float* s_const = reinterpret_cast<float*>(tmem_slot + 2);
   float* s_xch = s_const + 192;
+  uint64_t* xbar = reinterpret_cast<uint64_t*>(s_xch + 1024);
 
   const int warp = threadIdx.x >> 5, lane = threadIdx.x & 31;
   const uint32_t rank = cluster_ctarank();
@@ -495,6 +538,8 @@
   if (threadIdx.x == 0) {
     for (int s = 0; s < a.stages; ++s) { mbar_init(&full[s], 1); mbar_init(&empty[s], 1); }
     for (int j = 0; j < a.S; ++j) { mbar_init(&afull[j], 1); mbar_init(&aempty[j], 32); }
+    if (POOL == 1)
+      for (int i = 0; i < 64; ++i) mbar_init(&xbar[i], DIL);
     mbar_init(wfull, 1);
     asm volatile("fence.mbarrier_init.release.cluster;" ::: "memory");
   }
@@ -541,6 +586,7 @@
       asm volatile("prefetch.tensormap [%0];" ::"l"(reinterpret_cast<uint64_t>(&mapA)) : "memory");
       asm volatile("prefetch.tensormap [%0];" ::"l"(reinterpret_cast<uint64_t>(&mapW)) : "memory");
       asm volatile("prefetch.tensormap [%0];" ::"l"(reinterpret_cast<uint64_t>(&mapO)) : "memory");
+      if (POOL == 1) asm volatile("prefetch.tensormap [%0];" ::"l"(reinterpret_cast<uint64_t>(&mapO3)) : "memory");
       {
         const uint32_t lbar = smem_u32(wfull) & 0xFEFFFFFFu;
         if (rank == 0) mbar_expect_tx(wfull, (uint32_t)(2 * w_bytes));
@@ -642,16 +688,18 @@
     }
   } else {
     const int px = q4 * 32 + lane;
-    const bool issuer = threadIdx.x == 64;
+    const bool qissuer = grp == 0 && lane == 0;
     const int trow = POOL == 2 ? px >> 1 : px;
     const bool writer = POOL == 2 ? !(lane & 1) : true;
     const uint32_t row_off = (uint32_t)trow * 128u;
     const uint32_t sw = (uint32_t)(trow & 7);
     const uint32_t hi_chunk = (uint32_t)(c0 >> 3);
     uint32_t t = 0, e = 0, dj = 0, dph = 0;
-    uint32_t w_tfull = 0;
-    const bool timed = a.dbg != nullptr;
-    const long long tstart = a.dbg ? clock64() : 0;
+    bool pend = false;
+    uint32_t* w_tfull = tmem_slot + 1;
+    const bool timed = a.dbg != nullptr && threadIdx.x == 64;
+    if (timed) *w_tfull = 0u;
+    if (a.dbg && threadIdx.x == 64) a.dbg[blockIdx.x * 8 + 6] = (unsigned long long)clock64();
     constexpr bool STATS = POOL == 0 && DIL == 1;
     float st_s[STATS ? CW : 1], st_q[STATS ? CW : 1];
 #pragma unroll
@@ -666,17 +714,18 @@
       const uint32_t d = (j0 + 2u * (uint32_t)a.S - 2u - dj) % (uint32_t)a.S;
       if (t == 0 || d >= 3) {
         if (t > 0)
-          for (int h = 0; h < 2; ++h) sweep_drain<CW, true>(afull, aempty, dj, dph, a.S, a.bn, tcol, real, false, lane, v, timed, w_tfull);
+          for (int h = 0; h < 2; ++h) sweep_drain<CW, true>(afull, aempty, dj, dph, pend, a.S, a.bn, tcol, real, false, lane, v, timed, w_tfull);
+        sweep_release<true>(aempty, dj, pend, a.S, lane);
         dj = slot_back(j0, 2, a.S);
       } else {
-        for (uint32_t h = 0; h < d; ++h) sweep_drain<CW, true>(afull, aempty, dj, dph, a.S, a.bn, tcol, real, false, lane, v, timed, w_tfull);
-      }
-      for (int h = 0; h < 2; ++h) sweep_drain<CW, true>(afull, aempty, dj, dph, a.S, a.bn, tcol, real, false, lane, v, timed, w_tfull);
+        for (uint32_t h = 0; h < d; ++h) sweep_drain<CW, true>(afull, aempty, dj, dph, pend, a.S, a.bn, tcol, real, false, lane, v, timed, w_tfull);
+      }
+      for (int h = 0; h < 2; ++h) sweep_drain<CW, true>(afull, aempty, dj, dph, pend, a.S, a.bn, tcol, real, false, lane, v, timed, w_tfull);
       float hprev[CW];
 #pragma unroll
       for (int k = 0; k < CW; ++k) hprev[k] = 0.f;
       for (int m = 0; m < nrow; ++m, ++t) {
-        sweep_drain<CW, true>(afull, aempty, dj, dph, a.S, a.bn, tcol, real, true, lane, v, timed, w_tfull);
+        sweep_drain<CW, true>(afull, aempty, dj, dph, pend, a.S, a.bn, tcol, real, true, lane, v, timed, w_tfull);
         if (real) {
 #pragma unroll
           for (int k4 = 0; k4 < CW / 4; ++k4) {
@@ -692,30 +741,7 @@
 
         int r_out = q + DIL * (n0 + m);
         if (POOL == 1) {
-          if (real) {
-            float* xw = s_xch + (((t & 1) * 4 + grp) * 4 + q4) * 32;
-            if (lane < DIL) {
-#pragma unroll
-              for (int k4 = 0; k4 < CW / 4; ++k4)
-                *reinterpret_cast<float4*>(xw + lane * 16 + 4 * k4) = make_float4(v[4 * k4], v[4 * k4 + 1], v[4 * k4 + 2], v[4 * k4 + 3]);
-            }
-            asm volatile("bar.sync %0, 128;" ::"r"(1 + grp) : "memory");
-            const bool edge = lane >= 32 - DIL;
-            const float* xr = s_xch + (((t & 1) * 4 + grp) * 4 + ((q4 + 1) & 3)) * 32 + (edge ? (lane - (32 - DIL)) * 16 : 0);
-#pragma unroll
-            for (int k4 = 0; k4 < CW / 4; ++k4) {
-              const float4 x4 = *reinterpret_cast<const float4*>(xr + 4 * k4);
-              const float xs[4] = {x4.x, x4.y, x4.z, x4.w};
-#pragma unroll
-              for (int k = 0; k < 4; ++k) {
-                float nb = __shfl_down_sync(0xffffffffu, v[4 * k4 + k], DIL);
-                if (edge) nb = xs[k];
-                const float h = fmaxf(v[4 * k4 + k], nb);
-                v[4 * k4 + k] = fmaxf(h, hprev[4 * k4 + k]);
-                hprev[4 * k4 + k] = h;
-              }
-            }
-          }
+          if (real) sweep_pool1<CW, DIL>(v, hprev, s_xch, xbar, t, grp, q4, lane);
           if (m == 0) continue;
           r_out -= DIL;
         }
@@ -740,41 +766,20 @@
             }
           }
         }
-        uint8_t* ob = sOut + (e % (uint32_t)a.out_bufs) * OB_BYTES;
-        if (a.out_bufs == 1) {
-          if (issuer) asm volatile("cp.async.bulk.wait_group.read 0;" ::: "memory");
-          asm volatile("bar.sync 5, 512;" ::: "memory");
-        }
-        if (real) {
-          uint32_t hi[CW / 2], lo[CW / 2];
-#pragma unroll
-          for (int k = 0; k < CW / 2; ++k) split2(v[2 * k], v[2 * k + 1], hi[k], lo[k]);
-#pragma unroll
-          for (int c = 0; c < CW / 8; ++c) {
-            if (!writer) break;
-            *reinterpret_cast<uint4*>(ob + row_off + (((hi_chunk + c) ^ sw) << 4)) = make_uint4(hi[4 * c], hi[4 * c + 1], hi[4 * c + 2], hi[4 * c + 3]);
-            *reinterpret_cast<uint4*>(ob + 16384 + row_off + (((hi_chunk + c) ^ sw) << 4)) = make_uint4(lo[4 * c], lo[4 * c + 1], lo[4 * c + 2], lo[4 * c + 3]);
-          }
-          asm volatile("fence.proxy.async.shared::cta;" ::: "memory");
-        }
-        if (a.out_bufs == 2 && issuer) asm volatile("cp.async.bulk.wait_group.read 0;" ::: "memory");
-        asm volatile("bar.sync 6, 512;" ::: "memory");
-        if (issuer) {
-          tma_store_3d(&mapO, ob, 0, POOL == 2 ? w0 >> 1 : w0, r_out);
-          tma_store_3d(&mapO, ob + 16384, 64, POOL == 2 ? w0 >> 1 : w0, r_out);
-          asm volatile("cp.async.bulk.commit_group;" ::: "memory");
-        }
+        sweep_emit<CW, DIL, POOL, false>(v, sOut + (e % (uint32_t)a.out_bufs) * OB_BYTES, a.out_bufs, real, writer, row_off, sw, hi_chunk,
+                                         q4, qissuer, &mapO, &mapO3, (POOL == 2 ? w0 >> 1 : w0) + q4 * (POOL == 2 ? 16 : 32), r_out);
         ++e;
       }
     }
     if (t > 0)
-      for (int h = 0; h < 2; ++h) sweep_drain<CW, true>(afull, aempty, dj, dph, a.S, a.bn, tcol, real, false, lane, v, timed, w_tfull);
-    if (issuer) asm volatile("cp.async.bulk.wait_group 0;" ::: "memory");
+      for (int h = 0; h < 2; ++h) sweep_drain<CW, true>(afull, aempty, dj, dph, pend, a.S, a.bn, tcol, real, false, lane, v, timed, w_tfull);
+    sweep_release<true>(aempty, dj, pend, a.S, lane);
+    if (qissuer) asm volatile("cp.async.bulk.wait_group 0;" ::: "memory");
     if constexpr (STATS) {
       if (a.stats) sweep_stats_flush<CW>(st_s, st_q, s_xch, ew, c0, real, lane, a.stats);
     }
     if (a.dbg && threadIdx.x == 64) {
-      a.dbg[blockIdx.x * 8 + 5] = (unsigned long long)w_tfull; a.dbg[blockIdx.x * 8 + 6] = (unsigned long long)(clock64() - tstart);
+      a.dbg[blockIdx.x * 8 + 5] = (unsigned long long)*w_tfull; a.dbg[blockIdx.x * 8 + 6] = (unsigned long long)clock64() - a.dbg[blockIdx.x * 8 + 6];
       a.dbg[blockIdx.x * 8 + 7] = t;
     }
   }
@@ -886,12 +891,12 @@
 }
 
 template <int KSTEPS, int DIL, int POOL, int CW, bool LO64, bool OUT32>
-static int launch_sweep_t(sc_ctx* ctx, const CUtensorMap& mapA, const CUtensorMap& mapW, const CUtensorMap& mapO, const SweepArgs& a,
-                          size_t smem, cudaStream_t st) {
+static int launch_sweep_t(sc_ctx* ctx, const CUtensorMap& mapA, const CUtensorMap& mapW, const CUtensorMap& mapO, const CUtensorMap& mapO3,
+                          const SweepArgs& a, size_t smem, cudaStream_t st) {
   auto kern = conv_sweep_kernel<KSTEPS, DIL, POOL, CW, LO64, OUT32>;
   SC_TRY(ensure_smem_attr(ctx, reinterpret_cast<const void*>(kern), 227 * 1024));
   const int grid = a.n_items < ctx->sm_count ? a.n_items : ctx->sm_count;
-  kern<<<grid, 576, smem, st>>>(mapA, mapW, mapO, a);
+  kern<<<grid, 576, smem, st>>>(mapA, mapW, mapO, mapO3, a);
   ctx->launches++;
   SC_CUDA(cudaGetLastError());
   return SC_OK;
@@ -1011,7 +1016,8 @@
   const int slot = (in_fmt ? 1 : 2) * SW_SLOT_HALF;
   const int w_bytes = w.npanels * 6 * w.bn * 128;
   const int ob_bytes = out_fmt ? 16384 : 32768;
-  const int fixed = 1024 + w_bytes + SW_BAR_BYTES + 192 * 4 + 2 * 4 * 4 * 2 * 16 * 4;
+  const int xch_bytes = 2 * 4 * 4 * 2 * 16 * 4 + (pool == 1 ? 64 * 8 : 0);
+  const int fixed = 1024 + w_bytes + SW_BAR_BYTES + 192 * 4 + xch_bytes;
   a.out_bufs = 2;
   a.stages = (227 * 1024 - fixed - 2 * ob_bytes) / slot;
   if (a.stages < 3) {
@@ -1023,7 +1029,7 @@
   SC_CHECK(use_pair || a.stages >= 2, SC_ERR_ARG, "conv_sweep: ring does not fit (layer %d)", layer);
   const size_t smem = (size_t)fixed + (size_t)a.stages * slot + (size_t)a.out_bufs * ob_bytes;
 
-  CUtensorMap mapA, mapW, mapO;
+  CUtensorMap mapA, mapW, mapO, mapO3;
   {
     const int pxe = in_fmt ? 64 : 128;
     cuuint64_t dims[3] = {(cuuint64_t)pxe, (cuuint64_t)Pw, (cuuint64_t)R};
@@ -1045,14 +1051,14 @@
                            CU_TENSOR_MAP_FLOAT_OOB_FILL_NONE);
     SC_CHECK(r == CUDA_SUCCESS, SC_ERR_CUDA, "conv_sweep: cuTensorMapEncodeTiled(W) failed with %d", (int)r);
   }
-  {
+  for (int m = 0; m < 2; ++m) {
     const int pxe = out_fmt ? 64 : 128;
     const int oPw = pool == 2 ? Pw / 2 : Pw, oR = pool == 2 ? R / 2 : R;
     cuuint64_t dims[3] = {(cuuint64_t)pxe, (cuuint64_t)oPw, (cuuint64_t)oR};
     cuuint64_t strides[2] = {(cuuint64_t)pxe * 2, (cuuint64_t)oPw * pxe * 2};
-    cuuint32_t box[3] = {64, (cuuint32_t)(pool == 2 ? 64 : a.strip_w), 1};
+    cuuint32_t box[3] = {64, (cuuint32_t)(pool == 2 ? 16 : (m == 1 && pool == 1) ? 32 - dil : 32), 1};
     cuuint32_t es[3] = {1, 1, 1};
-    CUresult r = s->encode(&mapO, CU_TENSOR_MAP_DATA_TYPE_BFLOAT16, 3, out, dims, strides, box, es,
+    CUresult r = s->encode(m ? &mapO3 : &mapO, CU_TENSOR_MAP_DATA_TYPE_BFLOAT16, 3, out, dims, strides, box, es,
                            CU_TENSOR_MAP_INTERLEAVE_NONE, CU_TENSOR_MAP_SWIZZLE_128B, CU_TENSOR_MAP_L2_PROMOTION_NONE,
                            CU_TENSOR_MAP_FLOAT_OOB_FILL_NONE);
     SC_CHECK(r == CUDA_SUCCESS, SC_ERR_CUDA, "conv_sweep: cuTensorMapEncodeTiled(O) failed with %d", (int)r);
@@ -1076,7 +1082,7 @@
     a.L = L; a.nseg = nseg;
     a.n_items = nsp * dil * nseg;
     const int wp_bytes = w.npanels * 3 * w.bn * 128;
-    const int fixed_p = 1024 + ((wp_bytes + 1023) & ~1023) + SW_BAR_BYTES + 192 * 4 + ((pool || stats) ? 2 * 4 * 4 * 2 * 16 * 4 : 0);
+    const int fixed_p = 1024 + ((wp_bytes + 1023) & ~1023) + SW_BAR_BYTES + 192 * 4 + ((pool || stats) ? xch_bytes : 0);
     a.out_bufs = 2;
     a.stages = (227 * 1024 - fixed_p - 2 * ob_bytes) / slot;
     if (a.stages < 3) { a.out_bufs = 1; a.stages = (227 * 1024 - fixed_p - ob_bytes) / slot; }
@@ -1099,23 +1105,23 @@
     if (dil == 1 && pool == 2) {
       auto kern = conv_sweep_pair_kernel<3, 1, 2>;
       SC_TRY(ensure_smem_attr(ctx, reinterpret_cast<const void*>(kern), 227 * 1024));
-      kern<<<2 * npairs, 576, smem_p, st>>>(mapA, mapWp, mapO, a);
+      kern<<<2 * npairs, 576, smem_p, st>>>(mapA, mapWp, mapO, mapO3, a);
     } else if (dil == 1 && !pool && w.ksteps == 4) {
       auto kern = conv_sweep_pair_kernel<4, 1, 0>;
       SC_TRY(ensure_smem_attr(ctx, reinterpret_cast<const void*>(kern), 227 * 1024));
-      kern<<<2 * npairs, 576, smem_p, st>>>(mapA, mapWp, mapO, a);
+      kern<<<2 * npairs, 576, smem_p, st>>>(mapA, mapWp, mapO, mapO3, a);
     } else if (dil == 1 && !pool) {
       auto kern = conv_sweep_pair_kernel<3, 1, 0>;
       SC_TRY(ensure_smem_attr(ctx, reinterpret_cast<const void*>(kern), 227 * 1024));
-      kern<<<2 * npairs, 576, smem_p, st>>>(mapA, mapWp, mapO, a);
+      kern<<<2 * npairs, 576, smem_p, st>>>(mapA, mapWp, mapO, mapO3, a);
     } else if (dil == 2 && pool == 1) {
       auto kern = conv_sweep_pair_kernel<3, 2, 1>;
       SC_TRY(ensure_smem_attr(ctx, reinterpret_cast<const void*>(kern), 227 * 1024));
-      kern<<<2 * npairs, 576, smem_p, st>>>(mapA, mapWp, mapO, a);
+      kern<<<2 * npairs, 576, smem_p, st>>>(mapA, mapWp, mapO, mapO3, a);
     } else if (dil == 4 && !pool) {
       auto kern = conv_sweep_pair_kernel<3, 4, 0>;
       SC_TRY(ensure_smem_attr(ctx, reinterpret_cast<const void*>(kern), 227 * 1024));
-      kern<<<2 * npairs, 576, smem_p, st>>>(mapA, mapWp, mapO, a);
+      kern<<<2 * npairs, 576, smem_p, st>>>(mapA, mapWp, mapO, mapO3, a);
     } else {
       set_error("conv_sweep: no pair kernel instance for dil=%d pool=%d", dil, pool);
       return SC_ERR_ARG;
@@ -1126,11 +1132,11 @@
   }
   SC_TRY(launch_item_flags(ctx, skip, a, a.nstrips, a.strip_w, dil, rows_out, st));
   ProfScope prof(ctx, prof_cls, st);
-  if (w.ksteps == 2 && dil == 1 && pool == 2 && i32 && o32 && w.bn == 32) return launch_sweep_t<2, 1, 2, 8, true, true>(ctx, mapA, mapW, mapO, a, smem, st);
-  if (w.ksteps == 2 && dil == 1 && pool == 1 && i32 && o32 && w.bn == 32) return launch_sweep_t<2, 1, 1, 8, true, true>(ctx, mapA, mapW, mapO, a, smem, st);
-  if (w.ksteps == 2 && dil == 2 && !pool && i32 && !o32) return launch_sweep_t<2, 2, 0, 16, true, false>(ctx, mapA, mapW, mapO, a, smem, st);
-  if (w.ksteps == 2 && dil == 1 && !pool && i32 && !o32) return launch_sweep_t<2, 1, 0, 16, true, false>(ctx, mapA, mapW, mapO, a, smem, st);
-  if (w.ksteps == 2 && dil == 1 && !pool && i32 && o32 && w.bn == 32) return launch_sweep_t<2, 1, 0, 8, true, true>(ctx, mapA, mapW, mapO, a, smem, st);
+  if (w.ksteps == 2 && dil == 1 && pool == 2 && i32 && o32 && w.bn == 32) return launch_sweep_t<2, 1, 2, 8, true, true>(ctx, mapA, mapW, mapO, mapO3, a, smem, st);
+  if (w.ksteps == 2 && dil == 1 && pool == 1 && i32 && o32 && w.bn == 32) return launch_sweep_t<2, 1, 1, 8, true, true>(ctx, mapA, mapW, mapO, mapO3, a, smem, st);
+  if (w.ksteps == 2 && dil == 2 && !pool && i32 && !o32) return launch_sweep_t<2, 2, 0, 16, true, false>(ctx, mapA, mapW, mapO, mapO3, a, smem, st);
+  if (w.ksteps == 2 && dil == 1 && !pool && i32 && !o32) return launch_sweep_t<2, 1, 0, 16, true, false>(ctx, mapA, mapW, mapO, mapO3, a, smem, st);
+  if (w.ksteps == 2 && dil == 1 && !pool && i32 && o32 && w.bn == 32) return launch_sweep_t<2, 1, 0, 8, true, true>(ctx, mapA, mapW, mapO, mapO3, a, smem, st);
   set_error("conv_sweep: no kernel instance for ksteps=%d dil=%d pool=%d in_fmt=%d out_fmt=%d", w.ksteps, dil, pool, in_fmt, out_fmt);
   return SC_ERR_ARG;
 }
```
